# firstBusiness/mathmap

Measured on AMD Instinct MI355X. Metric: Mpixels/sec (mandelbrot @8192x8192), higher is better.
Workload: dtype f32

## Files before the change

### include/mmhip.h

```cpp
#ifndef MMHIP_H
#define MMHIP_H

#include <stddef.h>
#include <stdint.h>

#ifdef __cplusplus
extern "C" {
#endif

typedef struct mmhip_filter mmhip_filter;
typedef struct mmhip_invocation mmhip_invocation;

enum { MMHIP_UV_INT = 0, MMHIP_UV_FLOAT = 1, MMHIP_UV_BOOL = 2, MMHIP_UV_COLOR = 3,
       MMHIP_UV_CURVE = 4, MMHIP_UV_GRADIENT = 5, MMHIP_UV_IMAGE = 6 };

enum { MMHIP_EDGE_COLOR = 0, MMHIP_EDGE_WRAP = 1, MMHIP_EDGE_REFLECT = 2, MMHIP_EDGE_ROTATE = 3 };

enum { MMHIP_GAUSS_EXACT = 0, MMHIP_GAUSS_TOLERANCE = 1 };

typedef struct mmhip_options {
    int intersample;
    int supersampling;
    int edge_behaviour_x, edge_behaviour_y;
    int tile_w;
    int specialize_uservals;
    int pixel_inc;
    int gauss_mode;
    int reserved[5];
} mmhip_options;

typedef struct mmhip_userval_info {
    int kind;
    int index;
    char name[64];
    int int_min, int_max, int_default;
    float float_min, float_max, float_default;
    int bool_default;
    unsigned image_flags;
} mmhip_userval_info;

const char *mmhip_last_error(void);
const char *mmhip_version(void);

void mmhip_default_options(mmhip_options *o);
mmhip_filter *mmhip_compile(const char *source, const mmhip_options *opts);
mmhip_filter *mmhip_compile_specialized(const char *source, const mmhip_options *opts, int n, const int *indices,
                                        const double *values);
mmhip_filter *mmhip_filter_specialized(const mmhip_filter *f, int n, const int *indices, const double *values);
mmhip_filter *mmhip_compile_ir_json(const char *ir_json, const mmhip_options *opts);
void mmhip_filter_free(mmhip_filter *f);
const char *mmhip_filter_name(const mmhip_filter *f);
int mmhip_filter_num_uservals(const mmhip_filter *f);
int mmhip_filter_userval_info(const mmhip_filter *f, int index, mmhip_userval_info *out);
const char *mmhip_filter_ir_json(mmhip_filter *f);
const char *mmhip_filter_ir_json_raw(mmhip_filter *f);
const char *mmhip_filter_kernel_source(mmhip_filter *f);
int mmhip_filter_gauss_mode(const mmhip_filter *f);
int mmhip_filter_num_native_calls(const mmhip_filter *f);
int mmhip_filter_builtin_ids(const mmhip_filter *f, char *buf, int cap);
enum { MMHIP_GEOMETRY_FIELDS = 13 };
int mmhip_filter_launch_geometry(const mmhip_filter *f, int region_w, int num_rows, int64_t *out);
int mmhip_filter_num_closures(const mmhip_filter *f);
int mmhip_filter_closure_launch_geometry(const mmhip_filter *f, int closure, int width, int height, int64_t *out);
int mmhip_filter_clip_launch_geometry(const mmhip_filter *f, int region_w, int num_rows, int frames, int64_t *out);
enum { MMHIP_CLIP_PLAN_FIELDS = 4 };
int mmhip_filter_clip_batch_plan(const mmhip_filter *f, int region_w, int num_rows, int frames, int64_t *out);
enum { MMHIP_CLIP_NATIVE_PLAN_FIELDS = 4 };
int mmhip_filter_clip_native_plan(const mmhip_filter *f, int region_w, int num_rows, int render_w, int render_h, int frames,
                                  int64_t *out);
const char *mmhip_filter_clip_kernel_source(mmhip_filter *f);
long mmhip_filter_jit_clip(mmhip_filter *f, int load_module);
long mmhip_filter_jit(mmhip_filter *f, int load_module);
double mmhip_filter_jit_seconds(const mmhip_filter *f);

mmhip_invocation *mmhip_invoke(mmhip_filter *f, int img_width, int img_height);
void mmhip_invocation_free(mmhip_invocation *inv);
int mmhip_set_int(mmhip_invocation *inv, int index, int value);
int mmhip_set_float(mmhip_invocation *inv, int index, float value);
int mmhip_set_bool(mmhip_invocation *inv, int index, int value);
int mmhip_set_color(mmhip_invocation *inv, int index, float r, float g, float b, float a);
int mmhip_set_native_row_margin(mmhip_invocation *inv, int margin);
int mmhip_set_curve(mmhip_invocation *inv, int index, const float *values1024);
int mmhip_set_gradient(mmhip_invocation *inv, int index, const uint32_t *rgba1024);
int mmhip_set_by_name(mmhip_invocation *inv, const char *name, const char *value);
int mmhip_set_image_host(mmhip_invocation *inv, int index, const uint8_t *pixels, int width, int height, int channels);
int mmhip_set_image_device(mmhip_invocation *inv, int index, const void *device_rgba32, int width, int height);
int mmhip_set_image_sequence_host(mmhip_invocation *inv, int index, const uint8_t *pixels, int width, int height, int channels,
                                  int num_frames);
int mmhip_set_image_sequence_device(mmhip_invocation *inv, int index, const void *device_rgba32, int width, int height,
                                    int num_frames);
enum { MMHIP_NATIVE_FRAME_ZERO = 0, MMHIP_NATIVE_FRAME_CURRENT = 1 };
int mmhip_set_native_input_frame(mmhip_invocation *inv, int mode);
int mmhip_set_edge_colors(mmhip_invocation *inv, uint32_t color_x, uint32_t color_y);
int mmhip_set_render_size(mmhip_invocation *inv, int render_width, int render_height);
int mmhip_set_sampling_offset(mmhip_invocation *inv, float offset_x, float offset_y);

int mmhip_render(mmhip_invocation *inv, int frame, float t, int region_x, int region_y, int region_w, int region_h,
                 int first_row, int last_row, void *out_device, int row_stride, int bpp, int floatmap, void *stream);
int mmhip_render_clip(mmhip_invocation *inv, int num_frames, const int *frames, const float *ts, int region_x, int region_y,
                      int region_w, int region_h, int first_row, int last_row, void *out_device, int row_stride,
                      int64_t frame_stride, int bpp, int floatmap, void *stream);
long mmhip_clip_batched_launches(mmhip_invocation *inv);
long mmhip_clip_prologue_frames(mmhip_invocation *inv);
long mmhip_clip_native_batches(mmhip_invocation *inv);
long mmhip_clip_native_blurs(mmhip_invocation *inv);
long mmhip_clip_native_direct_frames(mmhip_invocation *inv);
int mmhip_render_supersampled(mmhip_invocation *inv, int frame, float t, int region_x, int region_y, int region_w,
                              int region_h, void *out_device, int row_stride, int bpp, void *stream);
int mmhip_render_clip_supersampled(mmhip_invocation *inv, int num_frames, const int *frames, const float *ts,
                                   int region_x, int region_y, int region_w, int region_h, void *out_device, int row_stride,
                                   int64_t frame_stride, int bpp, void *stream);
long mmhip_clip_supersampled_batches(mmhip_invocation *inv);
enum { MMHIP_CLIP_SS_PLAN_FIELDS = 7 };
int mmhip_filter_clip_supersample_plan(const mmhip_filter *f, int region_w, int region_h, int bpp, int frames, int64_t *out);
int mmhip_render_host(mmhip_invocation *inv, int frame, float t, uint8_t *out_rgba);
int mmhip_sync(mmhip_invocation *inv);
int mmhip_enable_timing(mmhip_invocation *inv, int on);
double mmhip_last_kernel_ms(mmhip_invocation *inv);
int mmhip_drain_kernel_ms(mmhip_invocation *inv, double *out_ms, int cap);
int mmhip_drain_native_kernel_ms(mmhip_invocation *inv, char *names, double *out_ms, int cap);
long mmhip_direct_native_launches(mmhip_invocation *inv);
long mmhip_tolerance_blur_launches(mmhip_invocation *inv);

void *mmhip_device_alloc(size_t bytes);
void mmhip_device_free(void *p);
int mmhip_copy_to_host(void *dst_host, const void *src_device, size_t bytes);
int mmhip_copy_to_device(void *dst_device, const void *src_host, size_t bytes);
int mmhip_device_count(void);
int mmhip_set_device(int ordinal);

#ifdef __cplusplus
}
#endif
#endif
```

### mathmap_amd/_lib.py

```python
import ctypes as C
import os

_HERE = os.path.dirname(os.path.abspath(__file__))
LIB_PATH = os.path.join(_HERE, "libmathmap_hip.so")


class Options(C.Structure):
    _fields_ = [("intersample", C.c_int), ("supersampling", C.c_int),
                ("edge_behaviour_x", C.c_int), ("edge_behaviour_y", C.c_int),
                ("tile_w", C.c_int), ("specialize_uservals", C.c_int), ("pixel_inc", C.c_int),
                ("gauss_mode", C.c_int), ("reserved", C.c_int * 5)]


class UservalInfo(C.Structure):
    _fields_ = [("kind", C.c_int), ("index", C.c_int), ("name", C.c_char * 64),
                ("int_min", C.c_int), ("int_max", C.c_int), ("int_default", C.c_int),
                ("float_min", C.c_float), ("float_max", C.c_float), ("float_default", C.c_float),
                ("bool_default", C.c_int), ("image_flags", C.c_uint)]


SYMBOLS = {
    "mmhip_last_error": (C.c_char_p, []),
    "mmhip_version": (C.c_char_p, []),
    "mmhip_default_options": (None, [C.POINTER(Options)]),
    "mmhip_compile": (C.c_void_p, [C.c_char_p, C.POINTER(Options)]),
    "mmhip_compile_specialized": (C.c_void_p, [C.c_char_p, C.POINTER(Options), C.c_int, C.POINTER(C.c_int),
                                               C.POINTER(C.c_double)]),
    "mmhip_compile_ir_json": (C.c_void_p, [C.c_char_p, C.POINTER(Options)]),
    "mmhip_filter_specialized": (C.c_void_p, [C.c_void_p, C.c_int, C.POINTER(C.c_int), C.POINTER(C.c_double)]),
    "mmhip_filter_free": (None, [C.c_void_p]),
    "mmhip_filter_name": (C.c_char_p, [C.c_void_p]),
    "mmhip_filter_num_uservals": (C.c_int, [C.c_void_p]),
    "mmhip_filter_userval_info": (C.c_int, [C.c_void_p, C.c_int, C.POINTER(UservalInfo)]),
    "mmhip_filter_ir_json": (C.c_char_p, [C.c_void_p]),
    "mmhip_filter_ir_json_raw": (C.c_char_p, [C.c_void_p]),
    "mmhip_filter_kernel_source": (C.c_char_p, [C.c_void_p]),
    "mmhip_filter_gauss_mode": (C.c_int, [C.c_void_p]),
    "mmhip_filter_num_native_calls": (C.c_int, [C.c_void_p]),
    "mmhip_filter_builtin_ids": (C.c_int, [C.c_void_p, C.c_char_p, C.c_int]),
    "mmhip_filter_launch_geometry": (C.c_int, [C.c_void_p, C.c_int, C.c_int, C.POINTER(C.c_int64)]),
    "mmhip_filter_clip_launch_geometry": (C.c_int, [C.c_void_p, C.c_int, C.c_int, C.c_int, C.POINTER(C.c_int64)]),
    "mmhip_filter_clip_batch_plan": (C.c_int, [C.c_void_p, C.c_int, C.c_int, C.c_int, C.POINTER(C.c_int64)]),
    "mmhip_filter_clip_native_plan": (C.c_int, [C.c_void_p, C.c_int, C.c_int, C.c_int, C.c_int, C.c_int, C.POINTER(C.c_int64)]),
    "mmhip_filter_clip_kernel_source": (C.c_char_p, [C.c_void_p]),
    "mmhip_filter_jit_clip": (C.c_long, [C.c_void_p, C.c_int]),
    "mmhip_filter_num_closures": (C.c_int, [C.c_void_p]),
    "mmhip_filter_closure_launch_geometry": (C.c_int, [C.c_void_p, C.c_int, C.c_int, C.c_int, C.POINTER(C.c_int64)]),
    "mmhip_filter_jit": (C.c_long, [C.c_void_p, C.c_int]),
    "mmhip_filter_jit_seconds": (C.c_double, [C.c_void_p]),
    "mmhip_invoke": (C.c_void_p, [C.c_void_p, C.c_int, C.c_int]),
    "mmhip_invocation_free": (None, [C.c_void_p]),
    "mmhip_set_int": (C.c_int, [C.c_void_p, C.c_int, C.c_int]),
    "mmhip_set_float": (C.c_int, [C.c_void_p, C.c_int, C.c_float]),
    "mmhip_set_bool": (C.c_int, [C.c_void_p, C.c_int, C.c_int]),
    "mmhip_set_color": (C.c_int, [C.c_void_p, C.c_int, C.c_float, C.c_float, C.c_float, C.c_float]),
    "mmhip_set_native_row_margin": (C.c_int, [C.c_void_p, C.c_int]),
    "mmhip_set_native_input_frame": (C.c_int, [C.c_void_p, C.c_int]),
    "mmhip_drain_kernel_ms": (C.c_int, [C.c_void_p, C.c_void_p, C.c_int]),
    "mmhip_direct_native_launches": (C.c_long, [C.c_void_p]),
    "mmhip_tolerance_blur_launches": (C.c_long, [C.c_void_p]),
    "mmhip_drain_native_kernel_ms": (C.c_int, [C.c_void_p, C.c_char_p, C.c_void_p, C.c_int]),
    "mmhip_set_curve": (C.c_int, [C.c_void_p, C.c_int, C.c_void_p]),
    "mmhip_set_gradient": (C.c_int, [C.c_void_p, C.c_int, C.c_void_p]),
    "mmhip_set_by_name": (C.c_int, [C.c_void_p, C.c_char_p, C.c_char_p]),
    "mmhip_set_image_host": (C.c_int, [C.c_void_p, C.c_int, C.c_void_p, C.c_int, C.c_int, C.c_int]),
    "mmhip_set_image_device": (C.c_int, [C.c_void_p, C.c_int, C.c_void_p, C.c_int, C.c_int]),
    "mmhip_set_image_sequence_host": (C.c_int, [C.c_void_p, C.c_int, C.c_void_p, C.c_int, C.c_int, C.c_int, C.c_int]),
    "mmhip_set_image_sequence_device": (C.c_int, [C.c_void_p, C.c_int, C.c_void_p, C.c_int, C.c_int, C.c_int]),
    "mmhip_set_edge_colors": (C.c_int, [C.c_void_p, C.c_uint32, C.c_uint32]),
    "mmhip_set_render_size": (C.c_int, [C.c_void_p, C.c_int, C.c_int]),
    "mmhip_set_sampling_offset": (C.c_int, [C.c_void_p, C.c_float, C.c_float]),
    "mmhip_render": (C.c_int, [C.c_void_p, C.c_int, C.c_float, C.c_int, C.c_int, C.c_int, C.c_int,
                               C.c_int, C.c_int, C.c_void_p, C.c_int, C.c_int, C.c_int, C.c_void_p]),
    "mmhip_render_clip": (C.c_int, [C.c_void_p, C.c_int, C.POINTER(C.c_int), C.POINTER(C.c_float), C.c_int, C.c_int, C.c_int,
                                    C.c_int, C.c_int, C.c_int, C.c_void_p, C.c_int, C.c_int64, C.c_int, C.c_int, C.c_void_p]),
    "mmhip_clip_batched_launches": (C.c_long, [C.c_void_p]),
    "mmhip_clip_prologue_frames": (C.c_long, [C.c_void_p]),
    "mmhip_clip_native_batches": (C.c_long, [C.c_void_p]),
    "mmhip_clip_native_blurs": (C.c_long, [C.c_void_p]),
    "mmhip_clip_native_direct_frames": (C.c_long, [C.c_void_p]),
    "mmhip_render_supersampled": (C.c_int, [C.c_void_p, C.c_int, C.c_float, C.c_int, C.c_int, C.c_int, C.c_int,
                                            C.c_void_p, C.c_int, C.c_int, C.c_void_p]),
    "mmhip_render_clip_supersampled": (C.c_int, [C.c_void_p, C.c_int, C.POINTER(C.c_int), C.POINTER(C.c_float), C.c_int, C.c_int,
                                                 C.c_int, C.c_int, C.c_void_p, C.c_int, C.c_int64, C.c_int, C.c_void_p]),
    "mmhip_clip_supersampled_batches": (C.c_long, [C.c_void_p]),
    "mmhip_filter_clip_supersample_plan": (C.c_int, [C.c_void_p, C.c_int, C.c_int, C.c_int, C.c_int, C.POINTER(C.c_int64)]),
    "mmhip_render_host": (C.c_int, [C.c_void_p, C.c_int, C.c_float, C.c_void_p]),
    "mmhip_sync": (C.c_int, [C.c_void_p]),
    "mmhip_enable_timing": (C.c_int, [C.c_void_p, C.c_int]),
    "mmhip_last_kernel_ms": (C.c_double, [C.c_void_p]),
    "mmhip_device_alloc": (C.c_void_p, [C.c_size_t]),
    "mmhip_device_free": (None, [C.c_void_p]),
    "mmhip_copy_to_host": (C.c_int, [C.c_void_p, C.c_void_p, C.c_size_t]),
    "mmhip_copy_to_device": (C.c_int, [C.c_void_p, C.c_void_p, C.c_size_t]),
    "mmhip_device_count": (C.c_int, []),
    "mmhip_set_device": (C.c_int, [C.c_int]),
}

BACKEND_SYMBOLS = {
    "gen_and_load_hip_code": (C.c_void_p, [C.c_void_p, C.POINTER(C.c_void_p), C.c_char_p, C.c_char_p, C.c_void_p]),
    "unload_hip_code": (None, [C.c_void_p]),
    "mathmap_hip_set_get_pixel": (None, [C.c_void_p]),
    "mathmap_hip_invalidate_drawable": (None, [C.c_void_p]),
    "mathmap_hip_release_invocation": (None, [C.c_void_p]),
}

SELFTEST_SYMBOLS = {
    "mmhip_selftest_abi_roundtrip": (C.c_int, [C.c_char_p, C.c_int, C.c_void_p, C.c_int, C.c_int, C.c_int, C.c_int,
                                               C.c_int, C.c_float, C.c_int, C.c_void_p]),
    "mmhip_selftest_error": (C.c_char_p, []),
    "mmhip_selftest_set_pixel_inc": (None, [C.c_int]),
    "mmhip_selftest_eval_unary": (C.c_int, [C.c_int, C.c_uint, C.c_ulonglong, C.c_void_p]),
    "mmhip_selftest_eval_binary": (C.c_int, [C.c_int, C.c_ulonglong, C.c_ulonglong, C.c_void_p]),
    "mmhip_selftest_gauss_tolerance_map": (C.c_int, [C.c_void_p, C.c_int, C.c_int, C.c_float, C.c_float, C.c_void_p]),
    "mmhip_selftest_combine_ms": (C.c_long, [C.c_int, C.c_int, C.c_int, C.c_int, C.c_int, C.POINTER(C.c_double)]),
}
SELFTEST_PATH = os.path.join(_HERE, "libmathmap_hip_selftest.so")
_selftest = None


def selftest_lib():
    global _selftest
    if _selftest is None:
        lib()
        l = C.CDLL(SELFTEST_PATH, mode=C.RTLD_GLOBAL)
        for name, (res, args) in SELFTEST_SYMBOLS.items():
            fn = getattr(l, name)
            fn.restype = res
            fn.argtypes = args
        _selftest = l
    return _selftest

_lib = None


def lib():
    global _lib
    if _lib is None:
        if not os.path.exists(LIB_PATH):
            raise ImportError(
                "%s is missing: build it with `python -c 'import __graft_entry__ as g; g.build()'` "
                "or `make -C mathmap_amd/csrc` (there is no CPU fallback)" % LIB_PATH)
        l = C.CDLL(LIB_PATH)
# ... 7 lines not shown
```

### mathmap_amd/api.py

```python
import ctypes as C
import json

import numpy as np

from ._lib import Options, UservalInfo, lib

UV_INT, UV_FLOAT, UV_BOOL, UV_COLOR, UV_CURVE, UV_GRADIENT, UV_IMAGE = range(7)
GAUSS_MODES = {"exact": 0, "tolerance": 1}
NATIVE_INPUT_FRAMES = {"zero": 0, "current": 1}
EDGE_COLOR, EDGE_WRAP, EDGE_REFLECT, EDGE_ROTATE = range(4)
GEOMETRY_FIELDS = ("tiles_x", "tiles_y", "wg1", "nwg", "ppt", "tile_w", "tile_h", "unroll", "pair_mode", "single_pixel",
                   "xcd_order", "tiles_magic", "xcd_full")
CLIP_PLAN_FIELDS = ("grid_x", "frames_per_batch", "batches", "shared_slot")
CLIP_NATIVE_PLAN_FIELDS = ("eligible", "frames_per_batch", "batches", "bytes_per_frame")
CLIP_SS_PLAN_FIELDS = ("batched", "frames_per_batch", "batches", "bytes_per_frame", "long_pitch", "rows_per_item", "pixels_per_item")


class MathMapError(RuntimeError):
    pass


def _err():
    return lib().mmhip_last_error().decode("utf-8", "replace")

# ... 26 lines not shown
        if not self._h:
            raise MathMapError(_err())
        if constants:
            base, self._h = self._h, None
            try:
                self._h = self._specialized_handle(base, constants)
            finally:
                lib().mmhip_filter_free(base)

    @staticmethod
    def _specialized_handle(handle, constants):
        names = {}
        for i in range(lib().mmhip_filter_num_uservals(handle)):
            info = UservalInfo()
            lib().mmhip_filter_userval_info(handle, i, C.byref(info))
            names[info.name.decode()] = i
        for k in constants:
            if k not in names:
                raise MathMapError("filter has no user value `%s'" % k)
        idx = (C.c_int * len(constants))(*[names[k] for k in constants])
        val = (C.c_double * len(constants))(*[float(v) for v in constants.values()])
        h = lib().mmhip_filter_specialized(handle, len(constants), idx, val)
        if not h:
            raise MathMapError(_err())
        return h

    def __del__(self):
        h, self._h = getattr(self, "_h", None), None
        if h:
            lib().mmhip_filter_free(h)

    @property
    def name(self):
        return lib().mmhip_filter_name(self._h).decode()

    @property
    def uservals(self):
        out = []
        for i in range(lib().mmhip_filter_num_uservals(self._h)):
            info = UservalInfo()
            lib().mmhip_filter_userval_info(self._h, i, C.byref(info))
            out.append(dict(kind=info.kind, index=info.index, name=info.name.decode(),
                            int_min=info.int_min, int_max=info.int_max, int_default=info.int_default,
                            float_min=info.float_min, float_max=info.float_max, float_default=info.float_default,
                            bool_default=info.bool_default, image_flags=info.image_flags))
        return out

    @property
    def ir(self):
        return json.loads(lib().mmhip_filter_ir_json(self._h).decode())

    @property
    def ir_json(self):
        return lib().mmhip_filter_ir_json(self._h).decode()

    @property
    def ir_json_raw(self):
        return lib().mmhip_filter_ir_json_raw(self._h).decode()

    def specialized(self, values=None):
        consts = {}
        for u in self.uservals:
            if u["kind"] == UV_INT:
                consts[u["name"]] = u["int_default"]
            elif u["kind"] == UV_FLOAT:
                consts[u["name"]] = u["float_default"]
            elif u["kind"] == UV_BOOL:
                consts[u["name"]] = u["bool_default"]
        for k, v in (values or {}).items():
            if k in consts:
                consts[k] = v
        return Filter(self._source, _handle=self._specialized_handle(self._h, consts), **self._kwargs)

    @property
    def kernel_source(self):
        return lib().mmhip_filter_kernel_source(self._h).decode()

    @property
    def gauss_mode(self):
        mode = lib().mmhip_filter_gauss_mode(self._h)
        return {v: k for k, v in GAUSS_MODES.items()}[mode]

    @property
    def num_native_calls(self):
        return lib().mmhip_filter_num_native_calls(self._h)

    @property
    def builtin_ids(self):
        n = lib().mmhip_filter_builtin_ids(self._h, None, 0)
        buf = C.create_string_buffer(n)
        lib().mmhip_filter_builtin_ids(self._h, buf, n)
        return frozenset(buf.value.decode().split())

    def launch_geometry(self, region_w, num_rows, closure=None):
        out = (C.c_int64 * len(GEOMETRY_FIELDS))()
        if closure is None:
            rc = lib().mmhip_filter_launch_geometry(self._h, region_w, num_rows, out)
        else:
            rc = lib().mmhip_filter_closure_launch_geometry(self._h, closure, region_w, num_rows, out)
        if rc != 0:
            raise MathMapError(_err())
        return dict(zip(GEOMETRY_FIELDS, out))

    def clip_launch_geometry(self, region_w, num_rows, frames):
        out = (C.c_int64 * len(GEOMETRY_FIELDS))()
        if lib().mmhip_filter_clip_launch_geometry(self._h, region_w, num_rows, frames, out) != 0:
            raise MathMapError(_err())
        return dict(zip(GEOMETRY_FIELDS, out))

    def clip_batch_plan(self, region_w, num_rows, frames):
        out = (C.c_int64 * len(CLIP_PLAN_FIELDS))()
        if lib().mmhip_filter_clip_batch_plan(self._h, region_w, num_rows, frames, out) != 0:
            raise MathMapError(_err())
        return dict(zip(CLIP_PLAN_FIELDS, out))

    def clip_native_plan(self, region_w, num_rows, frames, render_w=None, render_h=None):
        out = (C.c_int64 * len(CLIP_NATIVE_PLAN_FIELDS))()
        rw, rh = region_w if render_w is None else render_w, num_rows if render_h is None else render_h
        if lib().mmhip_filter_clip_native_plan(self._h, region_w, num_rows, rw, rh, frames, out) != 0:
            raise MathMapError(_err())
        return dict(zip(CLIP_NATIVE_PLAN_FIELDS, out))

    def clip_supersample_plan(self, region_w, region_h, frames, bpp=4):
        out = (C.c_int64 * len(CLIP_SS_PLAN_FIELDS))()
        if lib().mmhip_filter_clip_supersample_plan(self._h, region_w, region_h, bpp, frames, out) != 0:
            raise MathMapError(_err())
        return dict(zip(CLIP_SS_PLAN_FIELDS, out))

    @property
    def clip_kernel_source(self):
        return lib().mmhip_filter_clip_kernel_source(self._h).decode()

    def jit_clip(self, load=False):
        n = lib().mmhip_filter_jit_clip(self._h, 1 if load else 0)
        if n < 0:
            raise MathMapError(_err())
        return n

    @property
    def num_closures(self):
        return lib().mmhip_filter_num_closures(self._h)

    def jit(self, load=False):
        n = lib().mmhip_filter_jit(self._h, 1 if load else 0)
        if n < 0:
            raise MathMapError(_err())
        return n

    @property
    def jit_seconds(self):
        return lib().mmhip_filter_jit_seconds(self._h)

    def invoke(self, width, height):
        return Invocation(self, width, height)


def as_image_sequence(array):
    a = np.ascontiguousarray(array, dtype=np.uint8)
    if a.ndim == 3:
        a = a[None]
    if a.ndim != 4 or a.shape[0] < 1:
        raise MathMapError("an image is [H,W,3|4], an image sequence [N,H,W,3|4] with N >= 1; got shape %s" % (tuple(np.shape(array)),))
    return a


class Invocation:
# ... 26 lines not shown
        u = self._index(name)
        k, i = u["kind"], u["index"]
        if k == UV_INT:
            self._check(lib().mmhip_set_int(self._h, i, int(value)))
        elif k == UV_FLOAT:
            self._check(lib().mmhip_set_float(self._h, i, float(value)))
        elif k == UV_BOOL:
            self._check(lib().mmhip_set_bool(self._h, i, int(bool(value))))
        elif k == UV_COLOR:
            r, g, b, a = value
            self._check(lib().mmhip_set_color(self._h, i, r, g, b, a))
        elif k == UV_IMAGE:
            self.set_image(name, value)
        else:
            raise MathMapError("cannot set user value `%s'" % name)

    def set_curve(self, name, values):
        u = self._index(name)
        a = np.ascontiguousarray(values, dtype=np.float32)
        if a.shape != (1024,):
            raise MathMapError("a curve has 1024 samples")
        self._check(lib().mmhip_set_curve(self._h, u["index"], a.ctypes.data_as(C.c_void_p)))

    def set_gradient(self, name, rgba):
        u = self._index(name)
        a = np.ascontiguousarray(rgba, dtype=np.uint32)
        if a.shape != (1024,):
            raise MathMapError("a gradient has 1024 samples")
        self._check(lib().mmhip_set_gradient(self._h, u["index"], a.ctypes.data_as(C.c_void_p)))

    def set_image(self, name, array):
        u = self._index(name)
        a = as_image_sequence(array)
        n, h, w, c = a.shape
        self._check(lib().mmhip_set_image_sequence_host(self._h, u["index"], a.ctypes.data_as(C.c_void_p), w, h, c, n))

    def set_image_device(self, name, device_ptr, width, height, keepalive=None, num_frames=1):
        u = self._index(name)
        self._check(lib().mmhip_set_image_sequence_device(self._h, u["index"], C.c_void_p(device_ptr), width, height, num_frames))
        if keepalive is not None:
            self._keep.append(keepalive)

    def set_native_row_margin(self, margin):
        self._check(lib().mmhip_set_native_row_margin(self._h, margin))

    def set_native_input_frame(self, mode):
        if mode not in NATIVE_INPUT_FRAMES:
            raise MathMapError("native input frame must be one of %s, not %r" % (", ".join(sorted(NATIVE_INPUT_FRAMES)), mode))
        self._check(lib().mmhip_set_native_input_frame(self._h, NATIVE_INPUT_FRAMES[mode]))

    def set_render_size(self, render_width, render_height):
        self._check(lib().mmhip_set_render_size(self._h, render_width, render_height))
        self.render_width, self.render_height = render_width, render_height

    def set_edge_colors(self, cx, cy):
        self._check(lib().mmhip_set_edge_colors(self._h, cx, cy))

    def enable_timing(self, on=True):
        self._check(lib().mmhip_enable_timing(self._h, 1 if on else 0))

    def last_kernel_ms(self):
        return lib().mmhip_last_kernel_ms(self._h)

    def drain_kernel_ms(self, cap=4096):
        buf = (C.c_double * cap)()
        n = lib().mmhip_drain_kernel_ms(self._h, buf, cap)
        if n < 0:
            raise MathMapError(_err())
        return [buf[i] for i in range(n)]

    def drain_native_kernel_ms(self, cap=4096):
        names = C.create_string_buffer(cap * 64)
        buf = (C.c_double * cap)()
        n = lib().mmhip_drain_native_kernel_ms(self._h, names, buf, cap)
        if n < 0:
            raise MathMapError(_err())
        return [(names.raw[i * 64:(i + 1) * 64].split(b"\0", 1)[0].decode(), buf[i]) for i in range(n)]

    def direct_native_launches(self):
        return lib().mmhip_direct_native_launches(self._h)

    def tolerance_blur_launches(self):
        return lib().mmhip_tolerance_blur_launches(self._h)

    def render(self, t=0.0, frame=0):
        out = np.empty((self.render_height, self.render_width, 4), dtype=np.uint8)
        self._check(lib().mmhip_render_host(self._h, frame, t, out.ctypes.data_as(C.c_void_p)))
        return out

    def render_rows(self, out_ptr, first_row, last_row, t=0.0, frame=0, row_stride=None, bpp=4, floatmap=False,
                    stream=0, region=None):
        rx, ry, rw, rh = region if region is not None else (0, 0, self.render_width, self.render_height)
        if row_stride is None:
            row_stride = rw * bpp
        self._check(lib().mmhip_render(self._h, frame, t, rx, ry, rw, rh, first_row, last_row, C.c_void_p(out_ptr),
                                       row_stride, bpp, 1 if floatmap else 0, C.c_void_p(stream)))

    def render_clip(self, num_frames=None, frames=None, ts=None, out_ptr=None, rows=None, region=None, row_stride=None,
                    frame_stride=None, bpp=4, floatmap=False, stream=0, supersample=False):
        from .striping import animation_frame_t
        if supersample and (floatmap or rows is not None):
            raise ValueError("render_clip: supersample=True renders whole regions of bytes: neither floatmap nor rows")
        if frames is None and ts is None:
            if num_frames is None:
                raise MathMapError("render_clip: give num_frames, or frames and ts")
            frames = list(range(num_frames))
            ts = [animation_frame_t(i, num_frames) for i in frames]
        elif frames is None or ts is None:
            raise MathMapError("render_clip: frames and ts go together")
        frames = np.ascontiguousarray(frames, dtype=np.int32).reshape(-1)
        ts = np.ascontiguousarray(ts, dtype=np.float32).reshape(-1)
        if num_frames is None:
            num_frames = len(frames)
        if len(frames) != num_frames or len(ts) != num_frames:
            raise MathMapError("render_clip: frames and ts must have num_frames = %d entries" % num_frames)
        rx, ry, rw, rh = region if region is not None else (0, 0, self.render_width, self.render_height)
        first_row, last_row = rows if rows is not None else (ry, ry + rh)
        fp, tp = frames.ctypes.data_as(C.POINTER(C.c_int)), ts.ctypes.data_as(C.POINTER(C.c_float))
        if supersample:
            return self._render_clip_supersampled(num_frames, fp, tp, out_ptr, (rx, ry, rw, rh), row_stride, frame_stride, bpp, stream)
        if out_ptr is not None:
            if row_stride is None:
                row_stride = rw * bpp
            if frame_stride is None:
                n_rows = max(min(last_row, ry + rh) - max(first_row, 0), 0)
                frame_stride = n_rows * (16 * self.render_width if floatmap else row_stride)
            self._check(lib().mmhip_render_clip(self._h, num_frames, fp, tp, rx, ry, rw, rh, first_row, last_row,
                                                C.c_void_p(out_ptr), row_stride, frame_stride, bpp, 1 if floatmap else 0,
                                                C.c_void_p(stream)))
            return None
        if rows is not None or region is not None or floatmap or bpp != 4 or row_stride is not None or frame_stride is not None:
            raise MathMapError("render_clip without out_ptr returns whole RGBA frames: pass out_ptr for bands, regions and other formats")
        out = np.empty((num_frames, self.render_height, self.render_width, 4), dtype=np.uint8)
        if num_frames < 1:
            raise MathMapError("render_clip: num_frames must be at least 1")
        dev = lib().mmhip_device_alloc(out.nbytes)
        if not dev:
            raise MathMapError(_err())
        try:
            self._check(lib().mmhip_render_clip(self._h, num_frames, fp, tp, rx, ry, rw, rh, first_row, last_row,
                                                C.c_void_p(dev), rw * 4, rw * 4 * rh, 4, 0, None))
            self.sync()
            self._check(lib().mmhip_copy_to_host(out.ctypes.data_as(C.c_void_p), C.c_void_p(dev), out.nbytes))
        finally:
            lib().mmhip_device_free(C.c_void_p(dev))
        return out

    def _render_clip_supersampled(self, num_frames, fp, tp, out_ptr, region, row_stride, frame_stride, bpp, stream):
        rx, ry, rw, rh = region
        if row_stride is None:
            row_stride = rw * bpp
        if frame_stride is None:
            frame_stride = rh * row_stride
        if out_ptr is not None:
            self._check(lib().mmhip_render_clip_supersampled(self._h, num_frames, fp, tp, rx, ry, rw, rh, C.c_void_p(out_ptr),
                                                             row_stride, frame_stride, bpp, C.c_void_p(stream)))
            return None
        if row_stride != rw * bpp or frame_stride != rh * rw * bpp:
            raise MathMapError("render_clip without out_ptr returns packed frames: pass out_ptr for padded rows and frames")
        if num_frames < 1:
            raise MathMapError("render_clip: num_frames must be at least 1")
        out = np.empty((num_frames, rh, rw, bpp), dtype=np.uint8)
        dev = lib().mmhip_device_alloc(out.nbytes)
        if not dev:
            raise MathMapError(_err())
        try:
# ... 42 lines not shown
```

### mathmap_amd/csrc/hipgen.cpp

```cpp
#include <cmath>
#include <cstdio>
#include <cstdlib>
#include <cstring>
#include <map>
#include <set>
#include <sstream>
#include <stdexcept>

#include "front.h"
#include "hipgen_internal.h"

namespace mm {
namespace hipgen {

std::optional<int> env_int(const char *name) {
    const char *e = getenv(name);
    return e ? std::optional<int>(atoi(e)) : std::nullopt;
}

std::string vname(const Value *v) {
    char buf[64];
    snprintf(buf, sizeof buf, "v%d_%d", v->var->id, v->index);
    return buf;
}
// ... 295 lines not shown
                    collect_values(s->phis, sl, defs, uses);
                    use(s->cond);
                    collect_values(s->body, sl, defs, uses);
                    break;
                default: break;
            }
        }
    }

    template <class F> static void each_stmt(const Block &b, F f) {
        for (const Stmt *s : b) {
            if (!f(s)) continue;
            if (s->kind == Stmt::If) { each_stmt(s->then_, f); each_stmt(s->else_, f); }
            if (s->kind == Stmt::While) each_stmt(s->body, f);
        }
    }
    static bool is_op(const Stmt *s, const char *cname, size_t n = 0) {
        return s->kind == Stmt::Assign && s->rhs.kind == Rhs::Op && (n ? !strncmp(s->rhs.op->cname, cname, n) : !strcmp(s->rhs.op->cname, cname));
    }
    static bool uses_noise(const Block &b) {
        bool noise = false;
        each_stmt(b, [&](const Stmt *s) { noise = noise || is_op(s, "libnoise_", 9); return true; });
        return noise;
    }

    std::string site_desc(const Stmt *s) const {
        auto it = site_view.find(s);
        return it != site_view.end() ? it->second : vname(s->rhs.args[2].value) + "_desc";
    }
    const Stmt *find_fetched_result() const {
        if (!opt.intersample || knobs.no_fetched_result) return nullptr;
        const Stmt *fetch = nullptr;
        for (int i = 0; i < 4; ++i) {
            const Value *v = code.result[i];
            const Stmt *d = v ? v->def : nullptr;
            if (!d || d->kind != Stmt::Assign || d->parent || !d->in_pixel || d->rhs.kind != Rhs::Op || strcmp(d->rhs.op->cname, "TUPLE_NTH") ||
                d->rhs.args[0].kind != Primary::Val || d->rhs.args[1].kind != Primary::IntConst || d->rhs.args[1].i != i)
                return nullptr;
            const Stmt *f = d->rhs.args[0].value->def;
            if (!f || f->parent || !(hot_sites.count(f) || hot_frame_sites.count(f)) || (fetch && f != fetch)) return nullptr;
            fetch = f;
        }
        return fetch;
    }

    void find_hot_fetches(const Block &b, std::vector<std::string> &views, std::vector<std::string> &conds) {
        std::vector<const Stmt *> sites;
        each_stmt(b, [&](const Stmt *s) {
            if (s->in_pixel && is_op(s, "ORIG_VAL") && s->rhs.args.size() == 4 && s->rhs.args[2].kind == Primary::Val && preloaded_desc.count(s->rhs.args[2].value))
                sites.push_back(s);
            return s->in_pixel;
        });
        auto frame_const = [&](const Primary &f) { return f.is_const() || (f.kind == Primary::Val && transfer_off.count(f.value)); };
        std::map<const Value *, std::set<std::string>> frames_of;
        for (const Stmt *s : sites)
            if (frame_const(s->rhs.args[3])) frames_of[s->rhs.args[2].value].insert(prim(s->rhs.args[3], PIXEL));
        const bool frame_hot = knobs.frame_hot.value_or(1) != 0;
        for (const Stmt *s : sites) {
            const Primary &f = s->rhs.args[3];
            const std::string desc = vname(s->rhs.args[2].value) + "_desc";
            if (frame_const(f)) {
                hot_sites.insert(s);
                if (frames_of[s->rhs.args[2].value].size() > 1) {
                    const std::string view = "mm_fv" + std::to_string(site_view.size());
                    views.push_back("const mm_image_desc " + view + " = mm_frame_view(" + desc + ");");
                    site_view[s] = view;
                }
                conds.push_back("mm_fetch_is_hot(" + site_desc(s) + ", (int)(" + prim(f, PIXEL) + "))");
            } else if (frame_hot) {
                hot_frame_sites.insert(s);
                conds.push_back("mm_fetch_is_hot_any(" + desc + ")");
            }
        }
    }

    static bool hoisted_uses_time(const Block &b) {
        bool uses = false;
        each_stmt(b, [&](const Stmt *s) {
            uses = uses || (s->hoisted && s->kind == Stmt::Assign && s->rhs.kind == Rhs::Internal && (s->rhs.internal == "t" || s->rhs.internal == "frame"));
            return true;
        });
        return uses;
    }
    static void pixel_stats(const Block &b, int &stmts, int &fetches) {
        each_stmt(b, [&](const Stmt *s) { stmts += s->in_pixel; fetches += s->in_pixel && is_op(s, "ORIG_VAL"); return s->in_pixel; });
    }

    int auto_unroll() const {
        if (knobs.unroll && *knobs.unroll >= 1 && *knobs.unroll <= 8) return *knobs.unroll;
        if (pixel_fetches == 0) return 1;
        return pixel_stmts <= 64 ? 4 : pixel_stmts <= 400 ? 2 : 1;
    }
    int auto_tile_w() const { return pixel_fetches >= 1 && pixel_stmts <= 12 ? 64 : 16; }

    void find_natives(Block &b, int loop_depth = 0) {
        for (Stmt *s : b) {
            if (s->kind == Stmt::Assign) {
                bool native = (s->rhs.kind == Rhs::Closure && s->rhs.filter->kind == Filter::Native) ||
                              (s->rhs.kind == Rhs::Op && !strcmp(s->rhs.op->cname, "RENDER"));
                if (native) {
                    NativeCall nc;
                    nc.func = s->rhs.kind == Rhs::Closure ? s->rhs.filter->native_func : "RENDER";
                    for (const Primary &p : s->rhs.args) nc.arg_types.push_back(p.type());
                    nc.in_loop = loop_depth > 0;
                    native_index[s] = (int)ks.natives.size();
                    ks.natives.push_back(nc);
                }
            } else if (s->kind == Stmt::If) {
                find_natives(s->then_, loop_depth);
                find_natives(s->else_, loop_depth);
            } else if (s->kind == Stmt::While)
                find_natives(s->body, loop_depth + 1);
        }
    }

    void phis(Block &list, int branch, Slice sl, const std::string &ind) {
        auto src = [&](const Stmt *p) -> const Rhs & { return branch == 0 ? p->rhs : p->rhs2; };
        auto src_value = [&](const Stmt *p) { return src(p).kind == Rhs::Prim && src(p).prim.kind == Primary::Val ? src(p).prim.value : nullptr; };
        std::vector<Stmt *> mine;
        std::set<Value *> targets;
        for (Stmt *p : list)
            if (p->kind == Stmt::Phi && (sl == PROLOGUE ? p->hoisted : p->in_pixel) && src_value(p) != p->lhs) { mine.push_back(p); targets.insert(p->lhs); }
        bool hazard = false;
        for (Stmt *p : mine) hazard = hazard || targets.count(src_value(p)) > 0;
        if (!hazard) {
            for (Stmt *p : mine) out << ind << vname(p->lhs) << " = " << rhs(src(p), sl, p, p->lhs->var) << ";\n";
            return;
        }
        out << ind << "{\n";
        for (size_t i = 0; i < mine.size(); ++i)
            out << ind << "  " << ctype(mine[i]->lhs->var) << " pc" << i << " = "
                << rhs(src(mine[i]), sl, mine[i], mine[i]->lhs->var) << ";\n";
        for (size_t i = 0; i < mine.size(); ++i) out << ind << "  " << vname(mine[i]->lhs) << " = pc" << i << ";\n";
        out << ind << "}\n";
    }

    static bool is_sin_or_cos(const Stmt *s, bool *is_sin) {
        if (s->kind != Stmt::Assign || s->rhs.kind != Rhs::Op || s->rhs.args.size() != 1) return false;
        const char *cn = s->rhs.op->cname;
        if (strcmp(cn, "sin") && strcmp(cn, "cos")) return false;
        if (!s->lhs || s->lhs->var->type != Ty::Float || s->rhs.args[0].type() != Ty::Float || s->rhs.args[0].kind != Primary::Val)
            return false;
        *is_sin = !strcmp(cn, "sin");
        return true;
    }
    void join_sincos(Block &b) {
        for (size_t i = 0; i < b.size(); ++i) {
            bool sin_i, sin_j;
            Stmt *si = b[i];
            if (!si->in_pixel || sincos_role.count(si) || !is_sin_or_cos(si, &sin_i)) continue;
            for (size_t j = i + 1; j < b.size(); ++j) {
                Stmt *sj = b[j];
                if (!sj->in_pixel || sincos_role.count(sj) || !is_sin_or_cos(sj, &sin_j)) continue;
                if (sin_j == sin_i || sj->rhs.args[0].value != si->rhs.args[0].value) continue;
                sincos_role[si] = SinCosRole{sincos_ids, true};
                sincos_role[sj] = SinCosRole{sincos_ids, false};
                ++sincos_ids;
                break;
            }
        }
    }

    void stmts(Block &b, Slice sl, const std::string &ind) {
        if (opt.fast_math_exact && sl == PIXEL && sincos_scanned.insert(&b).second) join_sincos(b);
        for (Stmt *s : b) {
            bool mine = sl == PROLOGUE ? s->hoisted : sl == ROWS ? s->in_row : s->in_pixel;
// ... 285 lines not shown
}
struct mm_narg_t { int kind; int i; float f; mm_image img; };
MM_DEV mm_narg_t mm_narg(int v) { mm_narg_t a; a.kind = 0; a.i = v; a.f = (float)v; a.img = mm_null_image(); return a; }
MM_DEV mm_narg_t mm_narg(float v) { mm_narg_t a; a.kind = 1; a.i = (int)v; a.f = v; a.img = mm_null_image(); return a; }
MM_DEV mm_narg_t mm_narg(double v) { return mm_narg((float)v); }
MM_DEV mm_narg_t mm_narg(mm_image v) { mm_narg_t a; a.kind = 2; a.i = v.idx; a.f = 0.0f; a.img = v; return a; }
// Records a native-filter call for the host (which runs the filter's kernels between
// the prologue and the pixel kernel) and returns the handle of its result float map.
// ctr[0] counts the calls of this frame in the order they are made (the host runs them in that order).
MM_DEV mm_image mm_native_call(const mm_args &A, char *rec, int *ctr, int k, int nargs, mm_narg_t a0, mm_narg_t a1, mm_narg_t a2, mm_narg_t a3) {
    int *hdr = (int *)rec;
    hdr[0] = 1; hdr[1] = k; hdr[2] = nargs; hdr[3] = ctr[0]++;
    mm_narg_t *args = (mm_narg_t *)(rec + 16);
    args[0] = a0; args[1] = a1; args[2] = a2; args[3] = a3;
    mm_image im; im.idx = A.native_slot_base + k; im.pw = A.render_width; im.ph = A.render_height;
    im.xf = im.yf = 1.0f; im.resized = 0;
    return im;
}
// The same for a call site inside a loop: every call takes the next of the MM_NATIVE_DYN_CALLS dynamic entries behind
// the `sites' call sites (record, result slot); one call too many raises ctr[2] and the host refuses the frame.
MM_DEV mm_image mm_native_call_in_loop(const mm_args &A, char *dyn, int *ctr, int site, int sites, int nargs, mm_narg_t a0, mm_narg_t a1,
                                       mm_narg_t a2, mm_narg_t a3) {
    int n = ctr[1]++;
    if (n >= MM_NATIVE_DYN_CALLS) { ctr[2] = 1; n = MM_NATIVE_DYN_CALLS - 1; }
    mm_image im = mm_native_call(A, dyn + n * MM_NATIVE_REC_BYTES, ctr, site, nargs, a0, a1, a2, a3);
    im.idx = A.native_slot_base + sites + n;
    return im;
}
// (float) frame column / row of the pixel being evaluated (render_image's per-pixel loop, builtins.c:324-333)
#define __colF ((float)(col + A.region_x))
#define __rowF ((float)(rl + A.first_row))
#define MM_INTERNALS \
    const float t = A.t; const float R = A.R; const int frame = A.frame; \
    const int __canvasPixelW = A.img_width, __canvasPixelH = A.img_height; \
    const int __renderPixelW = A.render_width, __renderPixelH = A.render_height; \
    (void)t; (void)R; (void)frame; (void)__canvasPixelW; (void)__canvasPixelH; (void)__renderPixelW; (void)__renderPixelH;
)";
        if (ks.native_sites < (int)ks.natives.size())
            out << R"(// The pixel slice's side of a loop that runs in both slices: its n-th call from an in-loop site is the prologue's n-th.
MM_DEV mm_image mm_native_result_in_loop(const mm_args &A, int &n, int sites) {
    mm_image im; im.idx = A.native_slot_base + sites + (n < MM_NATIVE_DYN_CALLS ? n : MM_NATIVE_DYN_CALLS - 1); ++n;
    im.pw = A.render_width; im.ph = A.render_height; im.xf = im.yf = 1.0f; im.resized = 0;
    return im;
}
)";
    }

    void emit_functions() {
        FilterCode &root = fn_root ? *fn_root : code;
        if (root.functions.empty()) return;
        out << "#ifndef MM_MAX_CALL_DEPTH\n#define MM_MAX_CALL_DEPTH " << knobs.max_call_depth.value_or(16)
            << "\n#endif\n"
               "struct mm_uvarg { int i; float f; color_t c; mm_image img; };\n";
        auto head = [](size_t k) {
            return "template <int MM_D> __device__ __noinline__ mm_tup<4> mm_filter_" + std::to_string(k) +
                   "(const mm_args &A, const mm_uvarg *UV, float x, float y, float t, int col, int rl, unsigned &mm_rand_ctr)";
        };
        for (size_t k = 0; k < root.functions.size(); ++k) out << head(k) << ";\n";
        for (size_t k = 0; k < root.functions.size(); ++k) {
            FilterCode &fn = *root.functions[k];
            Generator g(fn, opt, knobs);
            g.fn_root = &root;
            g.in_function = true;
            std::vector<Value *> defs;
            std::set<Value *> uses;
            g.collect_values(fn.body, PIXEL, defs, uses);
            out << "// filter_" << (fn.filter ? fn.filter->name : "") << "\n" << head(k) << " {\n"
                   "  mm_tup<4> rt;\n  rt.v[0] = rt.v[1] = rt.v[2] = rt.v[3] = 0.0f;\n"
                   "  if constexpr (MM_D >= MM_MAX_CALL_DEPTH) { return rt; } else {\n"
                   "  const float R = A.R; const int frame = 0;      // new_template.c.in:379: filter_$name has `int frame = 0`\n"
                   "  const int __canvasPixelW = A.img_width, __canvasPixelH = A.img_height;\n"
                   "  const int __renderPixelW = A.render_width, __renderPixelH = A.render_height;\n"
                   "  (void)R; (void)frame; (void)__canvasPixelW; (void)__canvasPixelH; (void)__renderPixelW; (void)__renderPixelH;\n";
            g.decls(defs, "  ");
            g.stmts(fn.body, PIXEL, "  ");
            out << g.out.str();
            for (int i = 0; i < 4; ++i) out << "  rt.v[" << i << "] = " << g.prim(Primary::V(fn.result[i]), PIXEL) << ";\n";
            out << "  return rt;\n  }\n}\n";
        }
    }

    void emit_prologue_kernel() {
        ks.prologue_uses_time = hoisted_uses_time(code.body);
        ks.prologue_name = "mm_prologue";
        ks.pixel_name = "mm_pixels";
        auto tables = [](const std::string &first) {
            return "  {\n    const int gid = blockIdx.x * 256 + threadIdx.x;\n"
                   "    if (" + first + "gid < A.region_width) A.xtab[gid] = CALC_VIRTUAL_X(gid + A.region_x, A.frame_render_width, A.sampling_offset_x);\n"
                   "    if (" + first + "gid < A.num_rows) A.ytab[gid] = CALC_VIRTUAL_Y(A.first_row + gid, A.frame_render_height, A.sampling_offset_y);\n"
                   "    if (gid != 0) return;\n  }\n";
        };
        emit(KERNEL + "mm_prologue(mm_args A, char *XY) {\n" + tables(""),
             (ks.natives.empty() ? clip_prelude() : clip_prelude_natives()) + KERNEL + "mm_prologue_clip(mm_args A, char *XY, const mm_clip C) {\n  MM_CLIP_ENTRY\n" + tables("fi == 0 && "));
        out << "  MM_INTERNALS\n";
        if (!(fn_root ? fn_root : &code)->functions.empty()) out << "  const int col = 0, rl = 0; unsigned mm_rand_ctr = 0; (void)col; (void)rl; (void)mm_rand_ctr;\n";
        decls(pro_defs, "  ", true);
        if (!ks.natives.empty()) {
            for (const NativeCall &nc : ks.natives) out << "  *(int *)(XY + " << nc.record_offset << ") = 0;\n";
            out << "  { int *mm_ctr = (int *)(XY + " << ks.native_ctr_offset << "); mm_ctr[0] = mm_ctr[1] = mm_ctr[2] = mm_ctr[3] = 0; }\n";
        }
        stmts(code.body, PROLOGUE, "  ");
        for (Value *v : transfer_order)
            out << "  *(" << ctype(v->var) << " *)(XY + " << transfer_off[v] << ") = " << vname(v) << ";\n";
        out << "}\n\n";
    }

    void emit_rows_kernel() {
        emit(KERNEL + "mm_rows(mm_args A, const char *__restrict__ XY) {\n",
             KERNEL + "mm_rows_clip(mm_args A, const char *__restrict__ XY, const mm_clip C) {\n  MM_CLIP_ENTRY\n");
        out << "  const int rl = blockIdx.x * 256 + threadIdx.x;\n"
               "  if (rl >= A.num_rows) return;\n"
               "  MM_INTERNALS\n"
               "  const float y = A.ytab[rl];    // CALC_VIRTUAL_Y(first_row + rl, ...), by the prologue\n"
               "  (void)y;\n";
        transfer_loads(&row_uses);
        decls(row_defs, "  ");
        stmts(code.body, ROWS, "  ");
        for (size_t k = 0; k < row_transfer.size(); ++k) {
            Value *v = row_transfer[k];
            out << "  A.rowtab[" << k << " * A.num_rows + rl] = "
                << (v->var->type == Ty::Int ? "__int_as_float(" + vname(v) + ")" : vname(v)) << ";\n";
        }
        out << "}\n\n";
    }

    void emit_pixel_kernel() {
        if (knobs.waves_per_eu) out << "__attribute__((amdgpu_waves_per_eu(" << *knobs.waves_per_eu << "))) ";
        emit(KERNEL + "mm_pixels(mm_args A, const char *__restrict__ XY) {\n",
             KERNEL + "mm_pixels_clip(mm_args A, const char *__restrict__ XY, const mm_clip C) {\n"
                      "  if ((int)blockIdx.x >= C.nwg) return;      // padding workgroup\n  MM_CLIP_ENTRY\n");
        out << R"(  MM_INTERNALS
  // XCD-aware tile order (MM_XCD_ORDER, above): workgroups are dealt round-robin to the 8 XCDs; give each
  // XCD one contiguous band of tiles so neighbouring gathers share its L2 -- or, for a kernel that reads nothing,
  // take the tiles in dispatch order so that cheap and expensive regions of the frame are spread over all XCDs.
  const int tiles_x = (A.region_width + MM_TILE_W - 1) / MM_TILE_W;
)";
        emit("  const int nwg = gridDim.x;\n", "  const int nwg = C.nwg;      // the frame's workgroups (gridDim.x is padded)\n");
        out << R"(  const int bid = blockIdx.x;
#if MM_XCD_ORDER == 1
  const int xcd = bid & 7, q = bid >> 3;
  const int per = nwg >> 3, rem = nwg & 7;
  const int swz = xcd * per + (xcd < rem ? xcd : rem) + q;
#elif MM_XCD_ORDER == 2
  // runs of C = 2^m consecutive tiles (m: one tile row or a little more) dealt to the XCDs in turn: neighbours in a row
  // share an L2 like in a band, and every XCD gets runs from all over the frame; the last partial round keeps dispatch order
  const int m = 32 - __builtin_clz((unsigned)(tiles_x > 1 ? tiles_x - 1 : 1));
  const int full = (nwg >> (m + 3)) << (m + 3);
  const int q = bid >> 3;
  const int swz = bid < full ? ((((q >> m) << 3) + (bid & 7)) << m) + (q & ((1 << m) - 1)) : bid;
#else
  const int swz = bid;
  (void)nwg;
#endif
  const int tile_y = A.tiles_magic ? (int)__umulhi((unsigned)swz, A.tiles_magic) : swz / tiles_x, tile_x = swz - tile_y * tiles_x;
  const int col = tile_x * MM_TILE_W + (threadIdx.x % MM_TILE_W);
  // a workgroup owns MM_TILE_W x (MM_TILE_H * A.ppt) pixels; each work-item walks A.ppt rows
  // MM_TILE_H apart, so wave start-up (kernarg / descriptor loads, tile arithmetic) and the
  // dispatcher's per-workgroup cost are paid once per A.ppt pixels
  const int row0 = tile_y * (MM_TILE_H * A.ppt) + (threadIdx.x / MM_TILE_W);   // row within this launch
  if (col >= A.region_width) return;
  const float x = A.xtab[col];   // CALC_VIRTUAL_X(col + region_x, ...), once per column
  (void)x;
)";
        transfer_loads(nullptr);
        ks.single_pixel = knobs.single_pixel ? *knobs.single_pixel != 0 : pixel_stmts > 400 || transfer_order.size() > 24;
        if (ks.single_pixel) emit_single_pixel();
// ... 147 lines not shown
```

### mathmap_amd/csrc/hipgen.h

```cpp
#pragma once
#include <string>
#include <vector>

#include "ir.h"

namespace mm {

struct KernelOptions {
    int intersample = 1;
    int supersampling = 0;
    int edge_x = 0, edge_y = 0;
    int pixel_inc = 1;
    int tile_w = 0;
    int unroll = 0;
    bool hoist = true;
    bool fast_math_exact = true;
};

struct NativeCall {
    std::string func;
    std::vector<Ty> arg_types;
    int record_offset = 0;
    bool in_loop = false;
    bool dynamic = false;
};

enum { MM_NATIVE_REC_BYTES = 320, MM_NATIVE_ARG_BYTES = 32, MM_NATIVE_MAX_ARGS = 9, MM_NATIVE_DYN_CALLS = 16 };

struct KernelSource {
    std::string source;
    std::string prologue_name, pixel_name;
    int xy_bytes = 0;
    bool has_prologue = false;
    std::vector<NativeCall> natives;
    int native_sites = 0;
    int native_ctr_offset = -1;
    int tile_w = 16, tile_h = 16;
    int unroll = 1;
    bool prologue_uses_time = true;
    bool single_pixel = false;
    bool pair_mode = false;
    bool pair_exit = false;
    int xcd_order = 2;
    int row_values = 0;
    std::string rows_name;
    int direct_native = -1;
    std::string key;
    struct Splice { size_t begin, end; std::string text; };
    std::vector<Splice> clip_splices;
};

KernelSource generate_hip(FilterCode &code, const KernelOptions &opt, FilterCode *functions_of = nullptr);
bool pair_peel_enabled();
void clip_kernel_source(const KernelSource &ks, std::string *source, std::string *key);
const char *clip_prelude();
const char *clip_prelude_natives();
const char *device_prelude();
const char *device_noise_prelude();
const char *device_fastmath_prelude();
const char *noise_table_text();

}
```

### mathmap_amd/csrc/native_filters.h

```cpp
#pragma once
#include <hip/hip_runtime.h>

#include <string>
#include <vector>

#include "mm_host_abi.h"

namespace mm {

struct NativeEnv {
    int supersampling = 0;
    int edge_x = 0, edge_y = 0;
    uint32_t edge_color_x = 0, edge_color_y = 0;
};

struct NativeWorkspace {
    NativeEnv env;
    bool gauss_tolerance = false;
    void *scratch = nullptr;
    size_t scratch_bytes = 0;
    bool keep_tolerance_map = false;
    void *reserve(size_t bytes);
    void release();
    struct Timed { const char *name; hipEvent_t a, b; };
    bool timing = false;
    std::vector<Timed> timed;
    std::vector<std::pair<hipEvent_t, hipEvent_t>> timed_free;
    template <class F> void timed_launch(const char *name, hipStream_t s, F &&launch) {
        if (!timing || timed.size() >= 4096) { launch(); return; }
        Timed t{name, nullptr, nullptr};
        if (!timed_free.empty()) { t.a = timed_free.back().first; t.b = timed_free.back().second; timed_free.pop_back(); }
        else if (hipEventCreate(&t.a) != hipSuccess || hipEventCreate(&t.b) != hipSuccess) { launch(); return; }
        (void)hipEventRecord(t.a, s);
        launch();
        (void)hipEventRecord(t.b, s);
        timed.push_back(t);
    }
    void *fft_fwd = nullptr, *fft_inv = nullptr;
    int fft_w = 0, fft_h = 0, fft_batch = 0;
    bool fft_valid = false;
};

struct NativeDirectOut {
    void *out = nullptr;
    int row_stride = 0;
    int first_row = 0, num_rows = 0, region_x = 0, region_w = 0;
    bool skip_map = false;
    bool written = false;
    bool tolerance = false;
};

int run_native_filter(const std::string &func, const HNativeRec &rec, const std::vector<HImageDesc> &images,
                      int render_w, int render_h, float *out_map, NativeWorkspace &ws, hipStream_t stream,
                      std::string *err, int *row_lo, int *row_hi,
                      NativeDirectOut *direct = nullptr);

bool gaussian_blur_batchable(const HNativeRec &rec, const HImageDesc *images, int num_images, int render_w, int render_h,
                             const NativeEnv &env, size_t *ckpt_bytes, size_t *map_bytes);
void gaussian_blur_batch_job_bytes(int render_w, int render_h, size_t *ckpt_bytes, size_t *map_bytes);
struct GaussClipJob {
    HNativeRec rec;
    const HImageDesc *images;
    int num_images;
    double *ckpt;
    float *mapT;
    float *out_map;
    unsigned char *pack_out;
};
struct GaussClipLaunch {
    int render_w = 0, render_h = 0;
    const NativeDirectOut *direct = nullptr;
    bool write_map = true;
};
size_t gaussian_blur_batch_table_bytes(size_t jobs);
struct GaussClipGroup { bool drawable; unsigned jobs; const void *vertical, *horizontal; unsigned pitch; };
int gaussian_blur_batch_tables(const std::vector<GaussClipJob> &jobs, const GaussClipLaunch &launch, const NativeEnv &env,
                               char *host_table, const char *device_table, std::vector<GaussClipGroup> *groups, std::string *err);
int gaussian_blur_batch_launch(const std::vector<GaussClipGroup> &groups, const GaussClipLaunch &launch, NativeWorkspace &ws,
                               hipStream_t s, std::string *err);

int fft_native_filter(const std::string &func, const HNativeRec &rec, const std::vector<HImageDesc> &images, int render_w,
                      int render_h, float *out_map, NativeWorkspace &ws, hipStream_t stream, std::string *err);
int native_input_map(const char *who, const HImage &img, const std::vector<HImageDesc> &images, const NativeEnv &env, int w,
                     int h, float *dst, const float **map, hipStream_t s, std::string *err);
void fft_release_plans(NativeWorkspace &ws);
void launch_render_drawable(const HImageDesc &in, const HImage &img, const NativeEnv &env, float *dst, int w, int h, hipStream_t s);

void launch_supersample_combine(const unsigned char *longs, const unsigned char *shorts, unsigned char *out, int w, int h,
                                int bpp, int out_stride, hipStream_t s);
constexpr int SS_CLIP_ROWS = 8, SS_CLIP_PIXELS = 4;
size_t supersample_clip_long_pitch(int w, int bpp);
int64_t supersample_clip_items(int w, int h);
int launch_supersample_combine_clip(const unsigned char *longs, const unsigned char *shorts, unsigned char *out, int w, int h,
                                    int bpp, int row_stride, int64_t frame_stride, int frames, NativeWorkspace &ws, hipStream_t s,
                                    std::string *err);

}
```

### mathmap_amd/csrc/native_filters.hip

```cpp
#include "native_filters.h"
#include "mm_ss_combine.h"

#include <algorithm>
#include <cmath>
#include <cstring>
#include <type_traits>
#include <vector>

namespace mm {

void *NativeWorkspace::reserve(size_t bytes) {
    if (bytes > scratch_bytes) {
        if (scratch) (void)hipFree(scratch);
        scratch = nullptr;
        if (hipMalloc(&scratch, bytes) != hipSuccess) { scratch_bytes = 0; return nullptr; }
        scratch_bytes = bytes;
    }
    return scratch;
}

void NativeWorkspace::release() {
    fft_release_plans(*this);
    for (Timed &t : timed) timed_free.push_back({t.a, t.b});
    timed.clear();
// ... 671 lines not shown
}

__device__ __forceinline__ long fir_index(const FirArgs &g, int line, int k, int ch) {
    return g.vertical ? ((long)k * g.w + line) * 4 + ch : ((long)line * g.w + k) * 4 + ch;
}

__global__ void __launch_bounds__(256) k_fir_same(const float *__restrict__ in, int *__restrict__ flags, FirArgs g) {
    const long L = (long)blockIdx.x * 256 + threadIdx.x;
    const int lines = g.vertical ? g.w : g.h, n = g.vertical ? g.h : g.w;
    if (L >= (long)lines * 4) return;
    const int line = (int)(L >> 2), ch = (int)(L & 3);
    float last = in[fir_index(g, line, n - 1, ch)];
    int same = 0;
    for (int k = n - 1; k >= 0; --k) {
        const float c = in[fir_index(g, line, k, ch)];
        if (c == last) same++;
        else last = c;
    }
    flags[L] = same > (3 * n) / 4;
}

__global__ void __launch_bounds__(256) k_fir_apply(const float *__restrict__ in, float *__restrict__ out,
                                                   const int *__restrict__ flags, const float *__restrict__ curve,
                                                   const float *__restrict__ csum, FirArgs g) {
    const long e = (long)blockIdx.x * 256 + threadIdx.x;
    if (e >= (long)g.w * g.h * 4) return;
    const int ch = (int)(e & 3);
    const long px = e >> 2;
    const int col = (int)(px % g.w), row = (int)(px / g.w);
    const int line = g.vertical ? col : row, k = g.vertical ? row : col;
    const int n = g.vertical ? g.h : g.w;
    const int length = g.length;
    const float *c = curve + length, *cs = csum + length;
    auto pix = [&](int i) {
        int kk = k + i;
        kk = kk < 0 ? 0 : (kk >= n ? n - 1 : kk);
        return in[fir_index(g, line, kk, ch)];
    };
    float val = 0.0f;
    if (!flags[line * 4 + ch]) {
        val += pix(0) * c[0];
        for (int i = 1; i <= length; ++i) val += (pix(i) + pix(-i)) * c[i];
        val = val / g.total;
    } else {
        int pos = -length;
        auto runlen = [&](int p) {
            const float v = pix(p);
            int r = 1;
            while (k + p + r < n + length && pix(p + r) == v) ++r;
            return r;
        };
        float s1 = cs[-length];
        int nb = runlen(pos);
        int i = -length + nb;
        while (i <= length) {
            const int s2 = (int)cs[i];
            val += pix(pos) * (s2 - s1);
            s1 = (float)s2;
            pos += nb;
            nb = runlen(pos);
            i += nb;
        }
        val += pix(pos) * (cs[length] - s1);
        val = val / g.ctotal;
    }
    out[e] = val;
}

int gauss_rle(float *map, float *tmp, int w, int h, float hs, float vs, NativeWorkspace &ws, char *aux, hipStream_t s,
              std::string *err) {
    float *src = map, *dst = tmp;
    for (int pass = 0; pass < 2; ++pass) {
        const int vertical = pass == 0;
        const float sd = vertical ? vs : hs;
        if (!(sd > 0.0f)) continue;
        std::vector<float> curve, sum;
        int length;
        float total;
        make_rle_curve(sd, curve, sum, length, total);
        const int lines = vertical ? w : h;
        int *flags = (int *)aux;
        float *d_curve = (float *)(aux + (size_t)std::max(w, h) * 4 * sizeof(int));
        float *d_sum = d_curve + curve.size();
        if (hipMemcpyAsync(d_curve, curve.data(), curve.size() * 4, hipMemcpyHostToDevice, s) != hipSuccess ||
            hipMemcpyAsync(d_sum, sum.data(), sum.size() * 4, hipMemcpyHostToDevice, s) != hipSuccess ||
            hipStreamSynchronize(s) != hipSuccess) {
            *err = "gaussian_blur: tap upload failed";
            return -1;
        }
        FirArgs g{w, h, vertical, length, total, (int)total};
        k_fir_same<<<(unsigned)(((long)lines * 4 + 255) / 256), 256, 0, s>>>(src, flags, g);
        k_fir_apply<<<(unsigned)(((long)w * h * 4 + 255) / 256), 256, 0, s>>>(src, dst, flags, d_curve, d_sum, g);
        std::swap(src, dst);
    }
    if (src != map && hipMemcpyAsync(map, src, (size_t)w * h * 16, hipMemcpyDeviceToDevice, s) != hipSuccess) {
        *err = "gaussian_blur: copy failed";
        return -1;
    }
    (void)ws;
    return 0;
}

struct GaussPlan {
    const HImageDesc *in = nullptr;
    int w = 0, h = 0;
    float hs = 0.f, vs = 0.f;
    bool fir = false;
    bool identity = false;
    size_t ckpt_bytes = 0;
    size_t scratch_bytes = 0;
    size_t map_bytes = 0;
};

size_t checkpoint_bytes(int w, int h) {
    const size_t ck_v = (size_t)((h + IIR_U - 1) / IIR_U) * 4 * ((size_t)w * 4) * sizeof(double);
    const size_t ck_h = (size_t)((w + IIR_U - 1) / IIR_U) * 4 * ((size_t)h * 4) * sizeof(double);
    return std::max(ck_v, ck_h);
}

bool scan_offsets_fit(int w, int hn) { return (long)std::max(w, hn) * 4 * 20 * 8 < (1L << 32); }

int plan_gaussian_blur(const HNativeRec &rec, const HImageDesc *images, int num_images, int rw, int rh, const NativeEnv &env,
                       GaussPlan *p, std::string *err) {
    const HImage &img = rec.args[0].img;
    const float hdev = rec.args[1].f, vdev = rec.args[2].f;
    if (img.idx < 0 || img.idx >= num_images) { *err = "gaussian_blur: input is not a bitmap image"; return -1; }
    const HImageDesc &in = images[img.idx];
    p->in = &in;
    int w = rw, h = rh;
    if (in.kind == IMG_FLOATMAP) {
        w = in.w;
        h = in.h;
        if (w != rw || h != rh) { *err = "gaussian_blur: float-map input of a different size is not supported"; return -1; }
    } else if (in.kind != IMG_DRAWABLE) {
        *err = "gaussian_blur: input image is not bound";
        return -1;
    }
    p->w = w;
    p->h = h;
    const float ax = (float)((float)(w - 1) / 2.0);
    float ay = (float)((float)(h - 1) / 2.0);
    ay *= -1.0f;
    p->hs = (float)fabs(hdev * ax);
    p->vs = (float)fabs(vdev * ay);
    p->ckpt_bytes = checkpoint_bytes(w, h);
    p->scratch_bytes = ((p->ckpt_bytes + (size_t)std::max(w, h) * 64 + (size_t)(w + h) * sizeof(int) + 65536) + 255) & ~(size_t)255;
    p->map_bytes = (size_t)w * h * 4 * sizeof(float);
    p->fir = p->hs < 0.5f || p->vs < 0.5f;
    bool identity = !p->fir && in.kind == IMG_DRAWABLE && in.w == w && in.h == h;
    if (identity) {
        const float ax = (float)((float)(w - 1) / 2.0), bx = ax;
        const float by = (float)((float)(h - 1) / 2.0);
        const float ay2 = (float)(by * -1.0);
        for (int i = 0; i < w && identity; ++i) {
            float x = ((float)i - bx) / ax;
            if (img.resized) x *= img.xf;
            x = (x + in.middle_x) * in.scale_x;
            if (!env.supersampling) x += 0.5;
            identity = (int)floor((double)x) == i;
        }
        for (int i = 0; i < h && identity; ++i) {
            float y = ((float)i - by) / ay2;
            if (img.resized) y *= img.yf;
            y = -((y - in.middle_y) * in.scale_y);
            if (!env.supersampling) y += 0.5;
            identity = (int)floor((double)y) == i;
// ... 387 lines not shown
```

### mathmap_amd/csrc/runtime.cpp

```cpp
#include <hip/hip_runtime.h>
#include <hip/hiprtc.h>
#include <sys/stat.h>
#include <unistd.h>

#include <algorithm>
#include <chrono>
#include <cmath>
#include <cstdio>
#include <cstdlib>
#include <cstring>
#include <fstream>
#include <map>
#include <memory>
#include <sstream>
#include <string>
#include <vector>

#include "../../include/mmhip.h"
#include "front.h"
#include "hipgen.h"
#include "mm_host_abi.h"
#include "native_filters.h"
#include "passes.h"
#include "runtime_internal.h"
// ... 104 lines not shown
mmhip_filter *mmhip_compile(const char *source, const mmhip_options *opts) { return compile_source(source, opts, nullptr); }

mmhip_filter *mmhip_compile_specialized(const char *source, const mmhip_options *opts, int n, const int *indices,
                                        const double *values) {
    Module probe;
    try {
        parse_module(probe, source);
    } catch (const std::exception &e) {
        g_err = e.what();
        return nullptr;
    }
    std::map<int, Primary> consts;
    for (int i = 0; i < n; ++i) {
        if (indices[i] < 0 || indices[i] >= (int)probe.main->uservals.size()) { g_err = "user value index out of range"; return nullptr; }
        const UservalInfo &u = probe.main->uservals[indices[i]];
        if (u.kind == UvKind::Float) consts[u.index] = Primary::F((float)values[i]);
        else if (u.kind == UvKind::Int || u.kind == UvKind::Bool) consts[u.index] = Primary::I((int)values[i]);
    }
    return compile_source(source, opts, &consts);
}

}

mmhip_filter *mmhip_filter_new_empty() { return new mmhip_filter(); }

bool mmhip_filter_finalize(mmhip_filter *f, const KernelOptions &ko, std::string *err) {
    try {
        f->code->filter = f->module.main;
        if (f->ir_json_raw.empty()) f->ir_json_raw = dump_ir(*f->code);
        optimize(*f->code);
        analyze_frame_constants(*f->code);
        for (auto &sub : f->code->closure_renders) {
            sub->filter = f->module.main;
            optimize(*sub);
            eliminate_dead_cycles(*sub);
            analyze_frame_constants(*sub);
        }
        for (auto &fn : f->code->functions) optimize(*fn);
        f->kopt = ko;
        f->ir_json = dump_ir(*f->code);
        f->ks = generate_hip(*f->code, ko);
        generate_closure_kernels(f, ko);
    } catch (const std::exception &e) {
        *err = e.what();
        return false;
    }
    return true;
}

extern "C" {

void mmhip_filter_free(mmhip_filter *f) {
    if (!f) return;
    for (auto &p : f->spec_cache) mmhip_filter_free(p.second);
    for (mmhip_closure_kernel &ck : f->closures) if (ck.mod) (void)hipModuleUnload(ck.mod);
    if (f->mod) (void)hipModuleUnload(f->mod);
    if (f->clip_mod) (void)hipModuleUnload(f->clip_mod);
    delete f;
}

const char *mmhip_filter_name(const mmhip_filter *f) { return f->module.main->name.c_str(); }
int mmhip_filter_num_uservals(const mmhip_filter *f) { return (int)f->module.main->uservals.size(); }

int mmhip_filter_userval_info(const mmhip_filter *f, int index, mmhip_userval_info *out) {
    const auto &uvs = f->module.main->uservals;
    if (index < 0 || index >= (int)uvs.size()) return fail("user value index out of range");
    const UservalInfo &u = uvs[index];
    memset(out, 0, sizeof *out);
    out->kind = (int)u.kind;
    out->index = u.index;
    snprintf(out->name, sizeof out->name, "%s", u.name.c_str());
    out->int_min = u.imin; out->int_max = u.imax; out->int_default = u.idef;
    out->float_min = u.fmin; out->float_max = u.fmax; out->float_default = u.fdef;
    out->bool_default = u.bdef;
    out->image_flags = u.image_flags;
    return 0;
}

const char *mmhip_filter_ir_json(mmhip_filter *f) { return f->ir_json.c_str(); }
const char *mmhip_filter_ir_json_raw(mmhip_filter *f) { return f->ir_json_raw.c_str(); }
const char *mmhip_filter_kernel_source(mmhip_filter *f) { return f->ks.source.c_str(); }
int mmhip_filter_gauss_mode(const mmhip_filter *f) { return f->opts.gauss_mode; }
int mmhip_filter_num_native_calls(const mmhip_filter *f) { return f->ks.native_sites; }

int mmhip_filter_builtin_ids(const mmhip_filter *f, char *buf, int cap) {
    std::string s;
    for (const std::string &id : f->module.resolved_ids) { s += id; s += '\n'; }
    if (buf && cap > 0) snprintf(buf, (size_t)cap, "%s", s.c_str());
    return (int)s.size() + 1;
}
double mmhip_filter_jit_seconds(const mmhip_filter *f) { return f->jit_seconds; }

static int jit_source(const KernelSource &ks, std::vector<char> &code_object) {
    if (!code_object.empty()) return 0;
    std::vector<std::string> extra;
    std::string extra_key;
    if (const char *e = getenv("MMHIP_HIPRTC_FLAGS")) {
        std::istringstream is(e);
        for (std::string w; is >> w;) { extra.push_back(w); extra_key += "_" + std::to_string(std::hash<std::string>()(w) & 0xffff); }
    }
    std::string path = cache_dir() + "/" + ks.key + "_o2" + extra_key + ".hsaco";
    std::ifstream in(path, std::ios::binary);
    const char *ov = getenv("MMHIP_SOURCE_OVERRIDE");
    const bool may_override = ov && !strncmp(ov, ks.key.c_str(), ks.key.size()) && ov[ks.key.size()] == ':';
    if (in && !getenv("MMHIP_NO_CACHE") && !may_override) code_object.assign(std::istreambuf_iterator<char>(in), std::istreambuf_iterator<char>());
    if (!code_object.empty()) return 0;
    std::string source = ks.source;
    bool overridden = false;
    if (const char *e = getenv("MMHIP_SOURCE_OVERRIDE")) {
        const std::string spec = e;
        const size_t c = spec.find(':');
        if (c != std::string::npos && spec.substr(0, c) == ks.key) {
            std::ifstream f(spec.substr(c + 1));
            if (!f) return fail("MMHIP_SOURCE_OVERRIDE: cannot read " + spec.substr(c + 1));
            source.assign(std::istreambuf_iterator<char>(f), std::istreambuf_iterator<char>());
            overridden = true;
        }
    }
    hiprtcProgram prog;
    if (hiprtcCreateProgram(&prog, source.c_str(), "mathmap_filter.hip", 0, nullptr, nullptr) != HIPRTC_SUCCESS)
        return fail("hiprtcCreateProgram failed");
    std::vector<const char *> opts = {"--offload-arch=gfx950", "-O3", "-ffp-contract=off", "-std=c++17", "-fno-slp-vectorize"};
    for (const std::string &w : extra) opts.push_back(w.c_str());
    hiprtcResult r = hiprtcCompileProgram(prog, (int)opts.size(), opts.data());
    if (r != HIPRTC_SUCCESS) {
        size_t n = 0;
        hiprtcGetProgramLogSize(prog, &n);
        std::string log(n, 0);
        if (n) hiprtcGetProgramLog(prog, &log[0]);
        hiprtcDestroyProgram(&prog);
        return fail("hiprtc compile failed:\n" + log);
    }
    size_t n = 0;
    hiprtcGetCodeSize(prog, &n);
    code_object.resize(n);
    hiprtcGetCode(prog, code_object.data());
    hiprtcDestroyProgram(&prog);
    if (overridden) return 0;
    std::string tmp = path + ".tmp" + std::to_string((int)getpid());
    std::ofstream o(tmp, std::ios::binary);
    if (o) {
        o.write(code_object.data(), (std::streamsize)code_object.size());
        o.close();
        rename(tmp.c_str(), path.c_str());
    }
    return 0;
}

static int load_kernels(const KernelSource &ks, const std::vector<char> &code_object, hipModule_t *mod, hipFunction_t *f_pix,
                        hipFunction_t *f_pro) {
    hipError_t e = hipModuleLoadData(mod, code_object.data());
    if (e != hipSuccess) return fail(std::string("hipModuleLoadData: ") + hipGetErrorString(e));
    e = hipModuleGetFunction(f_pix, *mod, ks.pixel_name.c_str());
    if (e != hipSuccess) return fail(std::string("hipModuleGetFunction(pixels): ") + hipGetErrorString(e));
    e = hipModuleGetFunction(f_pro, *mod, ks.prologue_name.c_str());
    if (e != hipSuccess) return fail(std::string("hipModuleGetFunction(prologue): ") + hipGetErrorString(e));
    return 0;
}

long mmhip_filter_jit(mmhip_filter *f, int load_module) {
    auto t0 = std::chrono::steady_clock::now();
    if (jit_source(f->ks, f->code_object) != 0) return -1;
    for (mmhip_closure_kernel &ck : f->closures)
        if (jit_source(ck.ks, ck.code_object) != 0) return -1;
    if (load_module && !f->loaded) {
        if (load_kernels(f->ks, f->code_object, &f->mod, &f->f_pix, &f->f_pro) != 0) return -1;
// ... 20 lines not shown
        f->clip_ks.pixel_name = "mm_pixels_clip";
    }
    return f->clip_ks;
}

const char *mmhip_filter_clip_kernel_source(mmhip_filter *f) { return clip_source(f).source.c_str(); }

long mmhip_filter_jit_clip(mmhip_filter *f, int load_module) {
    auto t0 = std::chrono::steady_clock::now();
    const mm::KernelSource &ks = clip_source(f);
    if (jit_source(ks, f->clip_code_object) != 0) return -1;
    if (load_module && !f->clip_loaded) {
        if (load_kernels(ks, f->clip_code_object, &f->clip_mod, &f->f_pix_clip, &f->f_pro_clip) != 0) return -1;
        if (f->ks.row_values > 0) {
            hipError_t e = hipModuleGetFunction(&f->f_rows_clip, f->clip_mod, ks.rows_name.c_str());
            if (e != hipSuccess) return fail(std::string("hipModuleGetFunction(rows): ") + hipGetErrorString(e));
        }
        f->clip_loaded = true;
    }
    f->jit_seconds += std::chrono::duration<double>(std::chrono::steady_clock::now() - t0).count();
    return (long)f->clip_code_object.size();
}

mmhip_invocation *mmhip_invoke(mmhip_filter *f, int img_width, int img_height) {
    if (img_width <= 0 || img_height <= 0) { fail("image size must be positive"); return nullptr; }
    if (mmhip_filter_jit(f, 1) < 0) return nullptr;
    std::unique_ptr<mmhip_invocation> inv(new mmhip_invocation());
    inv->f = f;
    inv->img_w = inv->render_w = img_width;
    inv->img_h = inv->render_h = img_height;
    const auto &uvs = f->module.main->uservals;
    inv->uv.resize(std::max<size_t>(uvs.size(), 1));
    inv->image_slot_of_uv.assign(uvs.size(), -1);
    HImageDesc null_desc{};
    null_desc.kind = IMG_NULL;
    for (const UservalInfo &u : uvs) {
        HUserval &v = inv->uv[u.index];
        v.i = 0;
        switch (u.kind) {
            case UvKind::Int: v.i = u.idef; break;
            case UvKind::Float: v.f = u.fdef; break;
            case UvKind::Bool: v.i = u.bdef ? 1 : 0; break;
            case UvKind::Color: v.c = 0x000000ffu; break;
            case UvKind::Curve: {
                v.i = (int)(inv->curves.size() / 1024);
                for (int i = 0; i < 1024; ++i) inv->curves.push_back((float)i / (float)(1024 - 1));
                break;
            }
            case UvKind::Gradient: {
                v.i = (int)(inv->gradients.size() / 1024);
                for (int i = 0; i < 1024; ++i) {
                    float g = (float)i / (float)(1024 - 1);
                    uint32_t q = (uint32_t)(int)(g * 255.0) & 0xff;
                    inv->gradients.push_back((q << 24) | (q << 16) | (q << 8) | 255u);
                }
                break;
            }
            case UvKind::Image: {
                int slot = (int)inv->images.size();
                inv->image_slot_of_uv[u.index] = slot;
                inv->images.push_back(null_desc);
                v.image = slot;
                break;
            }
        }
    }
    inv->native_slot_base = (int)inv->images.size();
    inv->natives.resize(f->ks.natives.size());
    inv->images.resize(inv->images.size() + inv->natives.size(), null_desc);
    inv->closure_state.resize(f->closures.size());
    for (size_t c = 0; c < f->closures.size(); ++c) {
        auto &st = inv->closure_state[c];
        st.native_slot_base = (int)inv->images.size();
        st.native_results.resize(f->closures[c].ks.natives.size());
        inv->images.resize(inv->images.size() + st.native_results.size(), null_desc);
    }
    if (inv->images.empty()) inv->images.push_back(null_desc);
    auto bail = [&](const char *what, hipError_t e) -> mmhip_invocation * {
        fail(std::string(what) + ": " + hipGetErrorString(e));
        return nullptr;
    };
    hipError_t e;
    if ((e = hipStreamCreate(&inv->stream.s)) != hipSuccess) return bail("hipStreamCreate", e);
    if ((e = inv->d_uv.grow(inv->uv.size() * sizeof(HUserval))) != hipSuccess) return bail("hipMalloc", e);
    if ((e = inv->d_images.grow(inv->images.size() * sizeof(HImageDesc))) != hipSuccess) return bail("hipMalloc", e);
    if ((e = inv->d_curves.grow(inv->curves.size() * 4)) != hipSuccess) return bail("hipMalloc", e);
    if ((e = inv->d_gradients.grow(inv->gradients.size() * 4)) != hipSuccess) return bail("hipMalloc", e);
    const int xy_bytes = std::max(f->ks.xy_bytes, 256);
    if ((e = inv->launch.xy.grow(xy_bytes, DeviceBuffer::no_wait, true)) != hipSuccess) return bail("hipMalloc", e);
    return inv.release();
}

mmhip_invocation::~mmhip_invocation() {
    if (stream) (void)hipStreamSynchronize(stream);
    ws.release();
    for (auto &p : ev_pool) {
        (void)hipEventDestroy(p.first);
        (void)hipEventDestroy(p.second);
    }
}

void mmhip_invocation_free(mmhip_invocation *inv) { delete inv; }

static const UservalInfo *uv_info(mmhip_invocation *inv, int index, UvKind kind) {
    const auto &uvs = inv->f->module.main->uservals;
    if (index < 0 || index >= (int)uvs.size()) { fail("user value index out of range"); return nullptr; }
    if (uvs[index].kind != kind) { fail("user value `" + uvs[index].name + "' has a different type"); return nullptr; }
    return &uvs[index];
}

int mmhip_set_int(mmhip_invocation *inv, int index, int value) {
    const UservalInfo *u = uv_info(inv, index, UvKind::Int);
    if (!u) return -1;
    inv->uv[index].i = value;
    inv->tables_dirty = true;
    return 0;
}

int mmhip_set_float(mmhip_invocation *inv, int index, float value) {
    const UservalInfo *u = uv_info(inv, index, UvKind::Float);
    if (!u) return -1;
    inv->uv[index].f = value;
    inv->tables_dirty = true;
    return 0;
}

int mmhip_set_bool(mmhip_invocation *inv, int index, int value) {
    const UservalInfo *u = uv_info(inv, index, UvKind::Bool);
    if (!u) return -1;
    inv->uv[index].i = value ? 1 : 0;
    inv->tables_dirty = true;
    return 0;
}

int mmhip_set_color(mmhip_invocation *inv, int index, float r, float g, float b, float a) {
    const UservalInfo *u = uv_info(inv, index, UvKind::Color);
    if (!u) return -1;
    auto q = [](float v) { v = v < 0 ? 0 : v > 1 ? 1 : v; return (uint32_t)(v * 255.0); };
    inv->uv[index].c = (q(r) << 24) | (q(g) << 16) | (q(b) << 8) | q(a);
    inv->tables_dirty = true;
    return 0;
}

int mmhip_set_by_name(mmhip_invocation *inv, const char *name, const char *value) {
    for (const UservalInfo &u : inv->f->module.main->uservals) {
        if (u.name != name) continue;
        switch (u.kind) {
            case UvKind::Int: return mmhip_set_int(inv, u.index, atoi(value));
            case UvKind::Float: return mmhip_set_float(inv, u.index, (float)atof(value));
            case UvKind::Bool: return mmhip_set_bool(inv, u.index, atoi(value));
            default: return fail(std::string("user value `") + name + "' cannot be set from a string");
        }
    }
    return fail(std::string("filter has no user value `") + name + "'");
}

static void fill_drawable_desc(HImageDesc &d, const void *data, int w, int h, int num_frames) {
    d.data = data;
    d.w = w;
    d.h = h;
    d.kind = IMG_DRAWABLE;
    d.num_frames = num_frames;
    d.scale_x = (float)((w - 1) / 2.0);
    d.scale_y = (float)((h - 1) / 2.0);
    d.middle_x = 1.0f;
    d.middle_y = 1.0f;
    d.ax = d.bx = d.ay = d.by = 0.f;
}

static HImageDesc floatmap_desc(const void *data, int w, int h) {
    HImageDesc d{};
    d.data = data;
    d.w = w;
    d.h = h;
    d.kind = IMG_FLOATMAP;
    d.num_frames = 1;
    d.ax = d.bx = (float)((float)(w - 1) / 2.0);
    d.ay = d.by = (float)((float)(h - 1) / 2.0);
    d.ay *= -1.0f;
    return d;
}

static void input_changed(mmhip_invocation *inv) {
    inv->tables_dirty = true;
    ++inv->input_generation;
}

static bool sequence_bytes(int width, int height, int num_frames, size_t &bytes) {
    if (width < 0 || height < 0 || num_frames < 1) return false;
    size_t texels = 0;
    if ((uint64_t)height * (uint64_t)num_frames > (uint64_t)INT32_MAX) return false;
    return !__builtin_mul_overflow((size_t)width, (size_t)height, &texels) && !__builtin_mul_overflow(texels, (size_t)num_frames, &texels) &&
           !__builtin_mul_overflow(texels, (size_t)4, &bytes) && bytes <= (size_t)PTRDIFF_MAX;
}

int mmhip_set_image_sequence_device(mmhip_invocation *inv, int index, const void *device_rgba32, int width, int height, int num_frames) {
    if (num_frames < 1) return fail("num_frames must be at least 1");
    size_t bytes = 0;
    if (!sequence_bytes(width, height, num_frames, bytes)) return fail("image sequence: the size overflows (fewer than 2^31 rows in all, and a byte count that fits)");
    const UservalInfo *u = uv_info(inv, index, UvKind::Image);
    if (!u) return -1;
    int slot = inv->image_slot_of_uv[index];
    fill_drawable_desc(inv->images[slot], device_rgba32, width, height, num_frames);
    input_changed(inv);
    return 0;
}

int mmhip_set_image_device(mmhip_invocation *inv, int index, const void *device_rgba32, int width, int height) {
    return mmhip_set_image_sequence_device(inv, index, device_rgba32, width, height, 1);
}

}

void mmhip_unbind_image(mmhip_invocation *inv, const void *data) {
    for (HImageDesc &img : inv->images)
        if (img.data == data) {
            img.kind = IMG_NULL;
            img.data = nullptr;
            input_changed(inv);
        }
}

extern "C" {

int mmhip_set_image_sequence_host(mmhip_invocation *inv, int index, const uint8_t *pixels, int width, int height, int channels,
                                  int num_frames) {
    if (channels != 3 && channels != 4) return fail("channels must be 3 or 4");
    if (num_frames < 1) return fail("num_frames must be at least 1");
    size_t bytes = 0;
    if (!sequence_bytes(width, height, num_frames, bytes)) return fail("image sequence: the size overflows (fewer than 2^31 rows in all, and a byte count that fits)");
    if (!uv_info(inv, index, UvKind::Image)) return -1;
    const size_t n = (size_t)width * height;
    std::vector<uint32_t> packed;
    try { packed.resize(n); } catch (const std::bad_alloc &) { return fail("image sequence: out of host memory"); }
    DeviceBuffer d;
    HIP_TRY(d.grow(bytes));
    for (int k = 0; k < num_frames; ++k) {
        const uint8_t *frame = pixels + (size_t)k * n * channels;
        for (size_t i = 0; i < n; ++i) {
            const uint8_t *p = frame + i * channels;
            uint32_t a = channels == 4 ? p[3] : 255u;
            packed[i] = ((uint32_t)p[0] << 24) | ((uint32_t)p[1] << 16) | ((uint32_t)p[2] << 8) | a;
        }
        HIP_TRY(hipMemcpy((char *)d.get() + (size_t)k * n * 4, packed.data(), n * 4, hipMemcpyHostToDevice));
    }
    const void *old = inv->images[inv->image_slot_of_uv[index]].data;
    for (auto it = inv->owned.begin(); it != inv->owned.end(); ++it)
        if (it->get() == old) {
            (void)hipDeviceSynchronize();
            inv->owned.erase(it);
            break;
        }
    const void *dev = d.get();
    inv->owned.push_back(std::move(d));
    return mmhip_set_image_sequence_device(inv, index, dev, width, height, num_frames);
}

int mmhip_set_image_host(mmhip_invocation *inv, int index, const uint8_t *pixels, int width, int height, int channels) {
    return mmhip_set_image_sequence_host(inv, index, pixels, width, height, channels, 1);
}

int mmhip_set_curve(mmhip_invocation *inv, int index, const float *values1024) {
    if (!uv_info(inv, index, UvKind::Curve)) return -1;
    float *dst = &inv->curves[(size_t)inv->uv[index].i * 1024];
    if (memcmp(dst, values1024, 1024 * sizeof(float)) == 0) return 0;
    memcpy(dst, values1024, 1024 * sizeof(float));
    inv->tables_dirty = true;
    return 0;
}

int mmhip_set_gradient(mmhip_invocation *inv, int index, const uint32_t *rgba1024) {
    if (!uv_info(inv, index, UvKind::Gradient)) return -1;
    uint32_t *dst = &inv->gradients[(size_t)inv->uv[index].i * 1024];
    if (memcmp(dst, rgba1024, 1024 * sizeof(uint32_t)) == 0) return 0;
    memcpy(dst, rgba1024, 1024 * sizeof(uint32_t));
    inv->tables_dirty = true;
    return 0;
}

int mmhip_set_native_row_margin(mmhip_invocation *inv, int margin) {
    inv->native_row_margin = margin;
    return 0;
}

int mmhip_set_native_input_frame(mmhip_invocation *inv, int mode) {
    if (mode != MMHIP_NATIVE_FRAME_ZERO && mode != MMHIP_NATIVE_FRAME_CURRENT)
        return fail("native input frame: mode " + std::to_string(mode) + " is neither MMHIP_NATIVE_FRAME_ZERO (0) nor MMHIP_NATIVE_FRAME_CURRENT (1)");
    if (inv->native_input_frame != mode) ++inv->input_generation;
    inv->native_input_frame = mode;
    return 0;
}

int mmhip_set_edge_colors(mmhip_invocation *inv, uint32_t cx, uint32_t cy) {
    inv->edge_color_x = cx;
    inv->edge_color_y = cy;
    return 0;
}

int mmhip_set_render_size(mmhip_invocation *inv, int rw, int rh) {
    inv->render_w = rw;
    inv->render_h = rh;
    return 0;
}

int mmhip_set_sampling_offset(mmhip_invocation *inv, float ox, float oy) {
    inv->sampling_offset_x = ox;
    inv->sampling_offset_y = oy;
    return 0;
}

int mmhip_enable_timing(mmhip_invocation *inv, int on) {
    inv->timing = on != 0;
    inv->ws.timing = on != 0;
    return 0;
}

int mmhip_drain_native_kernel_ms(mmhip_invocation *inv, char *names, double *out_ms, int cap) {
    auto &tm = inv->ws.timed;
    if (!tm.empty() && hipEventSynchronize(tm.back().b) != hipSuccess) return fail("event sync failed");
    int n = 0;
    for (auto &t : tm) {
        float ms = 0;
        if (n < cap && hipEventElapsedTime(&ms, t.a, t.b) == hipSuccess) {
            snprintf(names + (size_t)n * 64, 64, "%s", t.name);
            out_ms[n++] = ms;
        }
        inv->ws.timed_free.push_back({t.a, t.b});
    }
    tm.clear();
    return n;
}

static int next_event_pair(mmhip_invocation *inv) {
    if (inv->ev_used == inv->ev_pool.size()) {
        if (inv->ev_pool.size() >= 4096) inv->ev_used = 0;
        else {
            hipEvent_t a, b;
            HIP_TRY(hipEventCreate(&a));
            HIP_TRY(hipEventCreate(&b));
            inv->ev_pool.push_back({a, b});
        }
    }
    inv->ev0 = inv->ev_pool[inv->ev_used].first;
    inv->ev1 = inv->ev_pool[inv->ev_used].second;
    ++inv->ev_used;
    return 0;
}

long mmhip_direct_native_launches(mmhip_invocation *inv) { return inv->direct_native_launches; }
long mmhip_tolerance_blur_launches(mmhip_invocation *inv) { return inv->tolerance_blur_launches; }

int mmhip_drain_kernel_ms(mmhip_invocation *inv, double *out_ms, int cap) {
    int n = 0;
    if (inv->ev_used > 0 && hipEventSynchronize(inv->ev_pool[inv->ev_used - 1].second) != hipSuccess) return fail("event sync failed");
    for (size_t i = 0; i < inv->ev_used && n < cap; ++i) {
        float ms = 0;
        if (hipEventElapsedTime(&ms, inv->ev_pool[i].first, inv->ev_pool[i].second) != hipSuccess) return fail("event elapsed failed");
        out_ms[n++] = ms;
    }
    inv->ev_used = 0;
    inv->ev_valid = false;
    return n;
}

double mmhip_last_kernel_ms(mmhip_invocation *inv) {
    if (!inv->ev_valid) return -1.0;
    if (hipEventSynchronize(inv->ev1) != hipSuccess) return -1.0;
    float ms = 0;
    if (hipEventElapsedTime(&ms, inv->ev0, inv->ev1) != hipSuccess) return -1.0;
    return ms;
}

static int upload_image_table(mmhip_invocation *inv, hipStream_t s) {
    HIP_TRY(hipStreamSynchronize(s));
    HIP_TRY(hipMemcpy(inv->d_images.get(), inv->images.data(), inv->images.size() * sizeof(HImageDesc), hipMemcpyHostToDevice));
    return 0;
}

static int upload_tables(mmhip_invocation *inv, hipStream_t s) {
    if (!inv->tables_dirty) return 0;
    if (upload_image_table(inv, s) != 0) return -1;
    HIP_TRY(hipMemcpy(inv->d_uv.get(), inv->uv.data(), inv->uv.size() * sizeof(HUserval), hipMemcpyHostToDevice));
    if (inv->d_curves) HIP_TRY(hipMemcpy(inv->d_curves.get(), inv->curves.data(), inv->curves.size() * 4, hipMemcpyHostToDevice));
    if (inv->d_gradients) HIP_TRY(hipMemcpy(inv->d_gradients.get(), inv->gradients.data(), inv->gradients.size() * 4, hipMemcpyHostToDevice));
    inv->tables_dirty = false;
    ++inv->table_generation;
    return 0;
}

struct LaunchGeometry {
    int tiles_x = 0, tiles_y = 0;
    long wg1 = 0;
    long nwg = 0;
    int ppt = 1;
    uint32_t tiles_magic = 0;
};

static int rows_per_item(long wgs) { return wgs >= 262144 ? 16 : wgs >= 131072 ? 8 : wgs >= 32768 ? 4 : wgs >= 8192 ? 2 : 1; }

static LaunchGeometry launch_geometry(const KernelSource &ks, int region_w, int num_rows) {
    LaunchGeometry g;
    g.tiles_x = (region_w + ks.tile_w - 1) / ks.tile_w;
    g.wg1 = (long)g.tiles_x * ((num_rows + ks.tile_h - 1) / ks.tile_h);
    int ppt = rows_per_item(g.wg1);
    if (const char *e = getenv("MMHIP_PPT")) ppt = std::max(1, atoi(e));
    if (ks.single_pixel) ppt = 1;
    const int u = std::max(1, ks.unroll);
    g.ppt = (ppt + u - 1) / u * u;
    g.tiles_y = (num_rows + ks.tile_h * g.ppt - 1) / (ks.tile_h * g.ppt);
    g.nwg = (long)g.tiles_x * g.tiles_y;
    g.tiles_magic = tile_division_magic(g.tiles_x, g.nwg);
    return g;
}

static LaunchGeometry clip_launch_geometry(const KernelSource &ks, int region_w, int num_rows, int frames) {
    LaunchGeometry g = launch_geometry(ks, region_w, num_rows);
    const int tile_rows = (num_rows + ks.tile_h - 1) / ks.tile_h;
    int ppt = std::min(rows_per_item(g.wg1 * std::max(frames, 1)), std::max(rows_per_item(g.wg1), tile_rows));
    if (const char *e = getenv("MMHIP_PPT")) ppt = std::max(1, atoi(e));
    if (ks.single_pixel) ppt = 1;
    const int u = std::max(1, ks.unroll);
    g.ppt = (ppt + u - 1) / u * u;
    g.tiles_y = (num_rows + ks.tile_h * g.ppt - 1) / (ks.tile_h * g.ppt);
    g.nwg = (long)g.tiles_x * g.tiles_y;
    g.tiles_magic = tile_division_magic(g.tiles_x, g.nwg);
    return g;
}

struct ClipPlan { long grid_x = 0; int max_frames = 0; };
static ClipPlan clip_plan(const LaunchGeometry &g) {
    static const int env_cap = [] {
        const char *e = getenv("MMHIP_CLIP_MAX_FRAMES");
        return e && atoi(e) > 0 ? atoi(e) : 65535;
    }();
    ClipPlan p;
    p.grid_x = (g.nwg + 7) / 8 * 8;
    const long by_items = ((1L << 23) - 1) / p.grid_x;
    p.max_frames = (int)std::min<long>(std::min(65535, env_cap), by_items);
    return p;
}

static int geometry_out(const KernelSource &ks, int region_w, int num_rows, int64_t *out, int clip_frames = 0) {
    if (region_w < 1 || num_rows < 1) return fail("launch geometry: empty region");
    const LaunchGeometry g = clip_frames > 0 ? clip_launch_geometry(ks, region_w, num_rows, clip_frames) : launch_geometry(ks, region_w, num_rows);
    int m = 0;
    for (unsigned v = (unsigned)(g.tiles_x > 1 ? g.tiles_x - 1 : 1); v; v >>= 1) ++m;
    const int64_t v[MMHIP_GEOMETRY_FIELDS] = {g.tiles_x, g.tiles_y, g.wg1, g.nwg, g.ppt, ks.tile_w, ks.tile_h, ks.unroll,
                                              ks.pair_mode, ks.single_pixel, ks.xcd_order, (int64_t)g.tiles_magic,
                                              (g.nwg >> (m + 3)) << (m + 3)};
    memcpy(out, v, sizeof v);
    return 0;
}

int mmhip_filter_launch_geometry(const mmhip_filter *f, int region_w, int num_rows, int64_t *out) {
    return geometry_out(f->ks, region_w, num_rows, out);
}

int mmhip_filter_clip_launch_geometry(const mmhip_filter *f, int region_w, int num_rows, int frames, int64_t *out) {
    if (frames < 1) return fail("clip launch geometry: num_frames must be at least 1");
    return geometry_out(f->ks, region_w, num_rows, out, frames);
}

int mmhip_filter_clip_batch_plan(const mmhip_filter *f, int region_w, int num_rows, int frames, int64_t *out) {
    if (frames < 1) return fail("clip batch plan: num_frames must be at least 1");
    if (region_w < 1 || num_rows < 1) return fail("clip batch plan: empty region");
    const bool batched = f->ks.natives.empty() && f->closures.empty();
    const ClipPlan p = clip_plan(clip_launch_geometry(f->ks, region_w, num_rows, frames));
    const int64_t per = batched ? p.max_frames : 0;
    const int64_t v[MMHIP_CLIP_PLAN_FIELDS] = {p.grid_x, per, per ? (frames + per - 1) / per : 0, !f->ks.prologue_uses_time};
    memcpy(out, v, sizeof v);
    return 0;
}

int mmhip_filter_num_closures(const mmhip_filter *f) { return (int)f->closures.size(); }

int mmhip_filter_closure_launch_geometry(const mmhip_filter *f, int closure, int width, int height, int64_t *out) {
    if (closure < 0 || closure >= (int)f->closures.size()) return fail("launch geometry: no such closure image");
    return geometry_out(f->closures[closure].ks, width, height, out);
}

static int grow_launch_buffers(LaunchBuffers &b, const KernelSource &ks, int region_w, int num_rows, bool rows, hipStream_t s) {
    auto wait = [s] { return hipStreamSynchronize(s); };
    HIP_TRY(b.xtab.grow((size_t)region_w * sizeof(float), wait));
    HIP_TRY(b.ytab.grow((size_t)num_rows * sizeof(float), wait));
    if (rows) HIP_TRY(b.rowtab.grow((size_t)ks.row_values * num_rows * sizeof(float), wait));
    HIP_TRY(b.xy.grow(std::max(ks.xy_bytes, 256), wait, true));
    return 0;
}

struct RecordedCall { size_t k; HNativeRec rec; const std::string *func; };
static int recorded_calls(const KernelSource &ks, const char *host, std::vector<RecordedCall> *calls) {
    calls->clear();
    if (ks.natives.empty()) return 0;
    int ctr[4];
    memcpy(ctr, host + ks.native_ctr_offset, sizeof ctr);
    if (ctr[2])
        return fail("native filters are called more than " + std::to_string((int)MM_NATIVE_DYN_CALLS) +
                    " times from inside a loop of the frame-constant code: not supported");
    for (size_t k = 0; k < ks.natives.size(); ++k) {
        RecordedCall c;
        c.k = k;
        memcpy(&c.rec, host + ks.natives[k].record_offset, sizeof c.rec);
        if (!c.rec.executed) continue;
        if (c.rec.index < 0 || c.rec.index >= ks.native_sites) return fail("internal: native call record names no call site");
        c.func = &ks.natives[c.rec.index].func;
        calls->push_back(c);
    }
    std::sort(calls->begin(), calls->end(), [](const RecordedCall &x, const RecordedCall &y) { return x.rec.pad < y.rec.pad; });
    return 0;
}

static bool same_native_call(const RecordedCall &c, const RecordedCall &m, const std::vector<int> &alias, int closure_slot_base) {
    if (*c.func != *m.func || c.rec.nargs != m.rec.nargs) return false;
    for (int i = 0; i < c.rec.nargs && i < 4; ++i) {
        const HNativeArg &x = c.rec.args[i], &y = m.rec.args[i];
        if (x.kind != y.kind) return false;
        if (x.kind != 2) {
            if (x.i != y.i || memcmp(&x.f, &y.f, sizeof x.f) != 0) return false;
            continue;
        }
        int idx = x.img.idx;
        const int rel = idx - closure_slot_base;
        if (rel >= 0 && rel < (int)alias.size()) {
            if (alias[rel] < 0) return false;
            idx = alias[rel];
        }
        if (idx != y.img.idx || x.img.pw != y.img.pw || x.img.ph != y.img.ph || x.img.resized != y.img.resized ||
            memcmp(&x.img.xf, &y.img.xf, sizeof x.img.xf) != 0 || memcmp(&x.img.yf, &y.img.yf, sizeof x.img.yf) != 0)
            return false;
    }
    return true;
}

static int render_closure(mmhip_invocation *inv, mmhip_filter *f, int cid, const HArgs &main_args, hipStream_t s,
                          const std::vector<RecordedCall> &main_done) {
    mmhip_closure_kernel &ck = f->closures[cid];
    auto &st = inv->closure_state[cid];
    const int w = main_args.render_width, h = main_args.render_height;
    if (st.map && (st.w != w || st.h != h)) {
        HIP_TRY(hipDeviceSynchronize());
        st.map.reset();
        for (DeviceBuffer &m : st.native_results) m.reset();
    }
    if (!st.map) {
        HIP_TRY(st.map.grow((size_t)w * h * 16));
        st.w = w;
        st.h = h;
    }
    if (grow_launch_buffers(st.launch, ck.ks, w, h, false, s) != 0) return -1;
    HArgs a = main_args;
    a.region_x = a.region_y = 0;
    a.region_width = w;
    a.region_height = h;
    a.sampling_offset_x = a.sampling_offset_y = 0.0f;
    a.first_row = 0;
    a.num_rows = h;
    a.output_bpp = 4;
    a.row_stride = w * 4;
    a.floatmap = 1;
    a.out = st.map.get();
    a.xtab = st.launch.xtab.get<float>();
    a.ytab = st.launch.ytab.get<float>();
    const LaunchGeometry geo = launch_geometry(ck.ks, w, h);
    a.ppt = geo.ppt;
    a.tiles_magic = geo.tiles_magic;
    char *xy = st.launch.xy.get<char>();
    void *params[] = {&a, &xy};
    const int n = std::max(w, h);
    a.native_slot_base = st.native_slot_base;
    HIP_TRY(hipModuleLaunchKernel(ck.f_pro, (unsigned)((n + 255) / 256), 1, 1, 256, 1, 1, 0, s, params, nullptr));
    if (!ck.ks.natives.empty()) {
        std::vector<char> host(ck.ks.xy_bytes);
        HIP_TRY(hipMemcpyAsync(host.data(), xy, host.size(), hipMemcpyDeviceToHost, s));
        HIP_TRY(hipStreamSynchronize(s));
        std::vector<RecordedCall> calls;
        if (recorded_calls(ck.ks, host.data(), &calls) != 0) return -1;
        std::vector<int> alias(ck.ks.natives.size(), -1);
        for (const RecordedCall &call : calls) {
            const size_t k = call.k;
            const HNativeRec &rec = call.rec;
            bool aliased = false;
            for (const RecordedCall &m : main_done) {
                const int mslot = inv->native_slot_base + (int)m.k;
                const NativeEntry &me = inv->natives[m.k];
                if (!same_native_call(call, m, alias, st.native_slot_base) || !me.map || inv->images[mslot].kind != IMG_FLOATMAP ||
                    inv->images[mslot].w != w || inv->images[mslot].h != h || me.rows.first > 0 || me.rows.second < h)
                    continue;
                inv->images[st.native_slot_base + (int)k] = inv->images[mslot];
                alias[k] = mslot;
                aliased = true;
                break;
            }
            if (aliased) continue;
            for (int i = 0; i < rec.nargs && i < 4; ++i)
                if (rec.args[i].kind == 2 && rec.args[i].img.idx <= -2)
                    return fail("a filter closure rendered for a native filter hands another closure to a native filter: not supported");
            HIP_TRY(st.native_results[k].grow((size_t)w * h * 16));
            std::string err;
            int lo = 0, hi = h;
            if (run_native_filter(*call.func, rec, inv->images, w, h, st.native_results[k].get<float>(), inv->ws, s, &err, &lo, &hi) != 0)
                return fail(err);
            inv->images[st.native_slot_base + (int)k] = floatmap_desc(st.native_results[k].get(), w, h);
        }
        if (upload_image_table(inv, s) != 0) return -1;
    }
    HIP_TRY(hipModuleLaunchKernel(ck.f_pix, (unsigned)geo.nwg, 1, 1, 256, 1, 1, 0, s, params, nullptr));
    return 0;
}

static bool direct_output_wanted(const mmhip_filter *f, const HArgs &a) {
    return f->ks.direct_native >= 0 && !a.floatmap && a.output_bpp == 4 && (a.row_stride & 3) == 0 && ((uintptr_t)a.out & 3) == 0 &&
           !getenv("MMHIP_NO_DIRECT_NATIVE");
}

static bool samples_own_pixels(const HArgs &a, const std::vector<float> &xt, const std::vector<float> &yt) {
    const HImageDesc m = floatmap_desc(nullptr, a.render_width, a.render_height);
    for (int c = 0; c < a.region_width; ++c)
        if (lrintf(m.ax * xt[c] + m.bx) != (long)a.region_x + c) return false;
    for (int r = 0; r < a.num_rows; ++r)
        if (lrintf(m.ay * yt[r] + m.by) != (long)a.first_row + r) return false;
    return true;
}

static int direct_output(const mmhip_filter *f, const HArgs &a, hipStream_t s, NativeDirectOut *direct) {
    const bool try_direct = direct_output_wanted(f, a);
    std::vector<float> xt, yt;
    if (try_direct) {
        xt.resize(a.region_width);
        yt.resize(a.num_rows);
        HIP_TRY(hipMemcpyAsync(xt.data(), a.xtab, xt.size() * sizeof(float), hipMemcpyDeviceToHost, s));
        HIP_TRY(hipMemcpyAsync(yt.data(), a.ytab, yt.size() * sizeof(float), hipMemcpyDeviceToHost, s));
    }
    HIP_TRY(hipStreamSynchronize(s));
    if (!try_direct) return 0;
    if (!samples_own_pixels(a, xt, yt)) return 0;
    direct->out = a.out;
    direct->row_stride = a.row_stride;
    direct->first_row = a.first_row;
    direct->num_rows = a.num_rows;
    direct->region_x = a.region_x;
    direct->region_w = a.region_width;
    return 0;
}

static int render_closure_args(mmhip_invocation *inv, mmhip_filter *f, const HArgs &a, hipStream_t s,
                               const std::vector<RecordedCall> &done, HNativeRec &rec, std::vector<HImageDesc> &images_k) {
    for (int i = 0; i < rec.nargs && i < 4; ++i) {
        HImage &img = rec.args[i].img;
        if (rec.args[i].kind != 2 || img.idx > -2) continue;
        const int cid = -2 - img.idx;
        if (cid >= (int)f->closures.size()) return fail("internal: closure image without a render kernel");
        if (render_closure(inv, f, cid, a, s, done) != 0) return -1;
        if (images_k.empty()) images_k = inv->images;
        img.idx = (int)images_k.size();
        img.pw = a.render_width;
        img.ph = a.render_height;
        img.xf = img.yf = 1.0f;
        img.resized = 0;
        images_k.push_back(floatmap_desc(inv->closure_state[cid].map.get(), a.render_width, a.render_height));
    }
    return 0;
}

enum { NO_FRAME_KEY = INT32_MIN };
static int view_sequence_args(const mmhip_invocation *inv, int frame, const std::string &func, const HNativeRec &rec,
                              std::vector<HImageDesc> &images_k, int *frame_key) {
    *frame_key = NO_FRAME_KEY;
    if (inv->native_input_frame != MMHIP_NATIVE_FRAME_CURRENT) return 0;
    for (int i = 0; i < rec.nargs && i < 4; ++i) {
        const int idx = rec.args[i].img.idx;
        if (rec.args[i].kind != 2 || idx < 0 || idx >= inv->native_slot_base) continue;
        const HImageDesc &d = inv->images[idx];
        if (d.kind != IMG_DRAWABLE || d.num_frames <= 1) continue;
        if (frame < 0 || frame >= d.num_frames)
            return fail((func == "RENDER" ? std::string("render()") : func.rfind("native_filter_", 0) == 0 ? func.substr(14) : func) + ": frame " + std::to_string(frame) + " is outside the input sequence (" + std::to_string(d.num_frames) +
                        " frames; native input frame mode `current')");
        if (images_k.empty()) images_k = inv->images;
        HImageDesc &v = images_k[idx];
        v.data = (const char *)d.data + (size_t)frame * d.w * d.h * 4;
        v.num_frames = 1;
        *frame_key = frame;
    }
    return 0;
}

static bool memo_hit(const mmhip_invocation *inv, const NativeEntry &e, const HNativeRec &rec, int frame_key, int want_lo, int want_hi,
                     std::vector<unsigned long long> *deps) {
    for (int i = 0; i < rec.nargs && i < 4; ++i)
        if (rec.args[i].kind == 2 && rec.args[i].img.idx >= inv->native_slot_base &&
            rec.args[i].img.idx < inv->native_slot_base + (int)inv->natives.size())
            deps->push_back(inv->natives[rec.args[i].img.idx - inv->native_slot_base].gen);
    return e.map && e.memo_gen == inv->input_generation && e.memo_frame == frame_key && memcmp(&e.memo, &rec, sizeof rec) == 0 && e.memo_deps == *deps &&
           e.rows.first <= want_lo && e.rows.second >= want_hi;
}

static void drop_native_map(mmhip_invocation *inv, size_t k, bool *table_changed) {
    NativeEntry &e = inv->natives[k];
    e.map.reset();
    e.memo_gen = e.seen_gen = ~0ULL;
    e.rows = {0, 0};
    HImageDesc &d = inv->images[inv->native_slot_base + (int)k];
    d.kind = IMG_NULL;
    d.data = nullptr;
    *table_changed = true;
}

static int run_natives(mmhip_invocation *inv, mmhip_filter *f, const HArgs &a, hipStream_t s, bool *direct_written) {
    std::vector<char> host(f->ks.xy_bytes);
    HIP_TRY(hipMemcpyAsync(host.data(), inv->launch.xy.get(), host.size(), hipMemcpyDeviceToHost, s));
    NativeDirectOut direct;
    if (direct_output(f, a, s, &direct) != 0) return -1;
    inv->ws.env.supersampling = f->kopt.supersampling;
    inv->ws.env.edge_x = f->kopt.edge_x;
    inv->ws.env.edge_y = f->kopt.edge_y;
    inv->ws.env.edge_color_x = inv->edge_color_x;
    inv->ws.env.edge_color_y = inv->edge_color_y;
    inv->ws.gauss_tolerance = f->opts.gauss_mode == MMHIP_GAUSS_TOLERANCE;
    int want_lo = 0, want_hi = a.render_height;
    if (inv->native_row_margin >= 0 && a.region_x == 0 && a.region_y == 0 && a.region_width == a.render_width &&
        a.region_height == a.render_height) {
        want_lo = std::max(0, a.first_row - inv->native_row_margin);
        want_hi = std::min(a.render_height, a.first_row + a.num_rows + inv->native_row_margin);
    }
    const bool whole = a.region_x == 0 && a.region_y == 0 && a.region_width == a.render_width &&
                       a.region_height == a.render_height && a.first_row == 0 && a.num_rows == a.render_height;
    bool table_changed = false;
    std::vector<RecordedCall> calls, done;
    if (recorded_calls(f->ks, host.data(), &calls) != 0) return -1;
    for (const RecordedCall &call : calls) {
        const size_t k = call.k;
        NativeEntry &e = inv->natives[k];
        HNativeRec rec = call.rec;
        if (e.map && (e.w != a.render_width || e.h != a.render_height)) {
            HIP_TRY(hipDeviceSynchronize());
            drop_native_map(inv, k, &table_changed);
        }
        std::vector<HImageDesc> images_k;
        if (render_closure_args(inv, f, a, s, done, rec, images_k) != 0) return -1;
        const bool closure_args = !images_k.empty();
        int frame_key = NO_FRAME_KEY;
        if (view_sequence_args(inv, a.frame, *call.func, rec, images_k, &frame_key) != 0) return -1;
        std::vector<unsigned long long> deps;
        if (memo_hit(inv, e, rec, frame_key, want_lo, want_hi, &deps) && !closure_args) {
            done.push_back(call);
            continue;
        }
        HIP_TRY(e.map.grow((size_t)a.render_width * a.render_height * 16));
        e.w = a.render_width;
        e.h = a.render_height;
        std::string err;
        int got_lo = want_lo, got_hi = want_hi;
        NativeDirectOut *dk = (direct.out && (int)k == f->ks.direct_native) ? &direct : nullptr;
        if (dk) {
            dk->skip_map = whole && !(e.seen_gen == inv->input_generation && e.seen_frame == frame_key && e.memo_deps == deps &&
                                      memcmp(&e.seen, &rec, sizeof rec) == 0);
            e.seen = rec;
            e.seen_frame = frame_key;
            e.seen_gen = inv->input_generation;
        }
        if (run_native_filter(*call.func, rec, images_k.empty() ? inv->images : images_k, a.render_width, a.render_height,
                              e.map.get<float>(), inv->ws, s, &err, &got_lo, &got_hi, dk) != 0)
            return fail(err);
        e.gen = ++inv->native_gen_counter;
        e.memo_deps = deps;
        if (dk && dk->written) *direct_written = true;
        if (dk && dk->written && dk->tolerance) ++inv->tolerance_blur_launches;
        if (dk && dk->written && dk->skip_map) {
            e.memo_gen = ~0ULL;
            e.rows = {0, 0};
            continue;
        }
        inv->images[inv->native_slot_base + (int)k] = floatmap_desc(e.map.get(), a.render_width, a.render_height);
        e.memo = rec;
        e.memo_frame = frame_key;
        e.memo_gen = inv->input_generation;
        e.rows = {got_lo, got_hi};
        table_changed = true;
        done.push_back(call);
    }
    if (f->ks.native_sites < (int)f->ks.natives.size()) {
        std::vector<char> used(f->ks.natives.size(), 0);
        for (const RecordedCall &call : calls) used[call.k] = 1;
        for (size_t k = (size_t)f->ks.native_sites; k < f->ks.natives.size(); ++k) {
            if (used[k] || !inv->natives[k].map) continue;
            HIP_TRY(hipStreamSynchronize(s));
            drop_native_map(inv, k, &table_changed);
        }
    }
    if (table_changed && upload_image_table(inv, s) != 0) return -1;
    return 0;
}

static void bake_uservals(Block &b, const std::map<int, Primary> &consts) {
    for (Stmt *st : b) {
        if (st->kind == Stmt::Assign && st->rhs.kind == Rhs::Op && st->rhs.args.size() == 1 &&
            st->rhs.args[0].kind == Primary::IntConst) {
            const char *n = st->rhs.op->cname;
            if (!strcmp(n, "USERVAL_INT_ACCESS") || !strcmp(n, "USERVAL_FLOAT_ACCESS") || !strcmp(n, "USERVAL_BOOL_ACCESS")) {
                auto it = consts.find(st->rhs.args[0].i);
                if (it != consts.end()) st->rhs = Rhs::P(it->second);
            }
        }
        if (st->kind == Stmt::If) { bake_uservals(st->then_, consts); bake_uservals(st->else_, consts); }
        if (st->kind == Stmt::While) bake_uservals(st->body, consts);
    }
}

static mmhip_filter *compile_ir_specialized(const mmhip_filter *f, const std::map<int, Primary> &consts, bool peel = true) {
    mmhip_filter *sp = mmhip_filter_new_empty();
    try {
        sp->code.reset(new FilterCode());
        load_ir_json(sp->module, *sp->code, (f->ir_json_raw.empty() ? f->ir_json : f->ir_json_raw).c_str());
        bake_uservals(sp->code->body, consts);
        specialize_constants(*sp->code);
        const bool peeled = peel && pair_peel_enabled() && peel_first_trips(*sp->code);
        for (auto &sub : sp->code->closure_renders) {
            bake_uservals(sub->body, consts);
            specialize_constants(*sub);
        }
        std::string err;
        if (!mmhip_filter_finalize(sp, f->kopt, &err)) throw CompileError(err);
        if (peeled && !sp->ks.pair_exit) {
            mmhip_filter_free(sp);
            return compile_ir_specialized(f, consts, false);
        }
        sp->opts = f->opts;
        sp->opts.specialize_uservals = 0;
    } catch (const std::exception &e) {
        g_err = e.what();
        mmhip_filter_free(sp);
        return nullptr;
    }
    return sp;
}

extern "C" mmhip_filter *mmhip_filter_specialized(const mmhip_filter *f, int n, const int *indices, const double *values) {
    std::map<int, Primary> consts;
    const auto &uvs = f->module.main->uservals;
    for (int i = 0; i < n; ++i) {
        if (indices[i] < 0 || indices[i] >= (int)uvs.size()) { g_err = "user value index out of range"; return nullptr; }
        const UservalInfo &u = uvs[indices[i]];
        if (u.kind == UvKind::Float) consts[u.index] = Primary::F((float)values[i]);
        else if (u.kind == UvKind::Int || u.kind == UvKind::Bool) consts[u.index] = Primary::I((int)values[i]);
    }
    mmhip_options o = f->opts;
    o.specialize_uservals = 0;
    return f->source.empty() ? compile_ir_specialized(f, consts) : compile_source(f->source.c_str(), &o, &consts);
}

static mmhip_filter *active_filter(mmhip_invocation *inv, int frame = 0, float t = 0.0f) {
    mmhip_filter *f = inv->f;
    if (!f->specialize || !f->ks.natives.empty() || (f->source.empty() && f->ir_json.empty() && f->ir_json_raw.empty())) return f;
    g_err.clear();
    const auto &uvs = f->module.main->uservals;
    std::string key;
    std::map<int, Primary> consts;
    for (const UservalInfo &u : uvs) {
        if (u.kind == UvKind::Int || u.kind == UvKind::Bool) consts[u.index] = Primary::I(inv->uv[u.index].i);
        else if (u.kind == UvKind::Float) consts[u.index] = Primary::F(inv->uv[u.index].f);
        else continue;
        key.append((const char *)&inv->uv[u.index], sizeof(HUserval));
    }
    if (consts.empty()) return f;
    auto it = f->spec_cache.find(key);
    if (it != f->spec_cache.end()) return it->second ? it->second : f;
    if (f->spec_min_uses > 1) {
        if (f->spec_uses.size() > 1024) f->spec_uses.clear();
        auto &u = f->spec_uses[key];
        if (u.count == 0 || u.frame != frame || u.t != t) {
            ++u.count;
            u.frame = frame;
            u.t = t;
        }
        if (u.count < f->spec_min_uses) return f;
    }
    f->spec_uses.erase(key);
    mmhip_options o = f->opts;
    o.specialize_uservals = 0;
    mmhip_filter *sp = f->source.empty() ? compile_ir_specialized(f, consts) : compile_source(f->source.c_str(), &o, &consts);
    if (sp && mmhip_filter_jit(sp, 1) < 0) { mmhip_filter_free(sp); sp = nullptr; }
    f->spec_cache[key] = sp;
    return sp ? sp : f;
}

static HArgs render_args(const mmhip_invocation *inv, int frame, float t, int region_x, int region_y, int region_w, int region_h,
                         int first_row, int last_row, void *out_device, int row_stride, int bpp, int floatmap) {
    HArgs a{};
    a.img_width = inv->img_w;
    a.img_height = inv->img_h;
    a.render_width = inv->render_w;
    a.render_height = inv->render_h;
    a.frame_render_width = inv->render_w;
    a.frame_render_height = inv->render_h;
    a.t = t;
    a.frame = frame;
    a.R = (float)sqrt(2.0);
    a.region_x = region_x;
    a.region_y = region_y;
    a.region_width = region_w;
    a.region_height = region_h;
    a.sampling_offset_x = inv->sampling_offset_x;
    a.sampling_offset_y = inv->sampling_offset_y;
    a.first_row = first_row;
    a.num_rows = last_row - first_row;
    a.output_bpp = bpp;
    a.row_stride = row_stride;
    a.floatmap = floatmap;
    a.edge_color_x = inv->edge_color_x;
    a.edge_color_y = inv->edge_color_y;
    a.uservals = inv->d_uv.get<HUserval>();
    a.images = inv->d_images.get<HImageDesc>();
    a.num_images = (uint32_t)inv->images.size();
    a.curves = inv->d_curves.get();
    a.gradients = inv->d_gradients.get();
    a.out = out_device;
    a.native_slot_base = inv->native_slot_base;
    return a;
}

int mmhip_render(mmhip_invocation *inv, int frame, float t, int region_x, int region_y, int region_w, int region_h,
                 int first_row, int last_row, void *out_device, int row_stride, int bpp, int floatmap, void *stream) {
    mmhip_filter *f = active_filter(inv, frame, t);
    hipStream_t s = stream ? (hipStream_t)stream : inv->stream;
    if (bpp < 1 || bpp > 4) return fail("output_bpp must be 1..4");
    if (region_w <= 0 || region_h <= 0) return fail("empty region");
    if (first_row < 0) first_row = 0;
    if (last_row > region_y + region_h) last_row = region_y + region_h;
    if (last_row <= first_row) return 0;
    if (upload_tables(inv, s) != 0) return -1;

    HArgs a = render_args(inv, frame, t, region_x, region_y, region_w, region_h, first_row, last_row, out_device, row_stride, bpp, floatmap);
    const size_t rowtab_bytes = inv->launch.rowtab.bytes;
    if (grow_launch_buffers(inv->launch, f->ks, region_w, a.num_rows, f->ks.row_values > 0, s) != 0) return -1;
    if (inv->launch.rowtab.bytes != rowtab_bytes) inv->pro_filter = nullptr;
    a.xtab = inv->launch.xtab.get<float>();
    a.ytab = inv->launch.ytab.get<float>();
    if (f->ks.row_values > 0) a.rowtab = inv->launch.rowtab.get<float>();
    char *xy = inv->launch.xy.get<char>();
    void *params[] = {&a, &xy};
    bool direct_written = false;
    {
        HArgs key = a;
        key.out = nullptr;
        key.row_stride = key.output_bpp = key.floatmap = key.ppt = 0;
        key.tiles_magic = 0;
        if (!f->ks.prologue_uses_time) { key.t = 0.0f; key.frame = 0; }
        const bool fresh = f->ks.natives.empty() && inv->pro_filter == f && inv->pro_stream == (void *)s &&
                           inv->pro_generation == inv->table_generation &&
                           memcmp(&key, &inv->pro_args, sizeof key) == 0;
        if (!fresh) {
            int n = std::max(region_w, a.num_rows);
            HIP_TRY(hipModuleLaunchKernel(f->f_pro, (unsigned)((n + 255) / 256), 1, 1, 256, 1, 1, 0, s, params, nullptr));
            if (f->ks.row_values > 0)
                HIP_TRY(hipModuleLaunchKernel(f->f_rows, (unsigned)((a.num_rows + 255) / 256), 1, 1, 256, 1, 1, 0, s, params, nullptr));
            if (!f->ks.natives.empty() && run_natives(inv, f, a, s, &direct_written) != 0) return -1;
            inv->pro_args = key;
            inv->pro_filter = f;
            inv->pro_stream = (void *)s;
            inv->pro_generation = inv->table_generation;
        }
    }
    const LaunchGeometry geo = launch_geometry(f->ks, region_w, a.num_rows);
    const long nwg = geo.nwg;
    if (nwg > 0x7fffffffL) return fail("region too large for one launch");
    a.ppt = geo.ppt;
    a.tiles_magic = geo.tiles_magic;
    if (inv->timing) {
        if (next_event_pair(inv) != 0) return -1;
        HIP_TRY(hipEventRecord(inv->ev0, s));
    }
    if (direct_written) ++inv->direct_native_launches;
    if (!direct_written) HIP_TRY(hipModuleLaunchKernel(f->f_pix, (unsigned)nwg, 1, 1, 256, 1, 1, 0, s, params, nullptr));
    if (inv->timing) {
        HIP_TRY(hipEventRecord(inv->ev1, s));
        inv->ev_valid = true;
    }
    return 0;
}

long mmhip_clip_batched_launches(mmhip_invocation *inv) { return inv->clip_batched_launches; }
long mmhip_clip_prologue_frames(mmhip_invocation *inv) { return inv->clip_prologue_frames; }
long mmhip_clip_native_batches(mmhip_invocation *inv) { return inv->clip_native_batches; }
long mmhip_clip_native_blurs(mmhip_invocation *inv) { return inv->clip_native_blurs; }
long mmhip_clip_native_direct_frames(mmhip_invocation *inv) { return inv->clip_native_direct_frames; }

struct HClipFrame { float t; int frame; };
struct HClip { const HClipFrame *frames; long long frame_stride; int xy_stride; int rowtab_stride; int nwg; int images_stride; };
static_assert(sizeof(HClip) == 32, "mm_clip layout");

static bool clip_native_eligible(const mmhip_filter *f, int native_row_margin) {
    if (f->ks.natives.empty() || f->ks.native_sites != (int)f->ks.natives.size() || !f->closures.empty()) return false;
    for (const NativeCall &nc : f->ks.natives)
        if (nc.func != "native_filter_gaussian_blur") return false;
    const char *seg = getenv("MMHIP_GAUSS_SEGMENTS");
    return f->opts.gauss_mode == MMHIP_GAUSS_EXACT && !(seg && *seg) && native_row_margin < 0;
}

struct ClipNativePlan { bool eligible = false; int per_batch = 0; size_t bytes_per_frame = 0; };
static ClipNativePlan clip_native_plan(const mmhip_filter *f, int native_row_margin, const ClipPlan &plan, int render_w, int render_h) {
    static const size_t budget = [] {
        const char *e = getenv("MMHIP_CLIP_NATIVE_BYTES");
        const long long v = e ? atoll(e) : 0;
        return v > 0 ? (size_t)v : (size_t)8 << 30;
    }();
    ClipNativePlan p;
    p.eligible = clip_native_eligible(f, native_row_margin);
    if (!p.eligible || render_w < 1 || render_h < 1) return p;
    size_t ck = 0, map = 0;
    gaussian_blur_batch_job_bytes(render_w, render_h, &ck, &map);
    p.bytes_per_frame = (size_t)f->ks.native_sites * (ck + 2 * map);
    const size_t by_bytes = budget / p.bytes_per_frame;
    const int per = (int)std::min<size_t>(std::min(plan.max_frames, 65535), by_bytes);
    p.per_batch = per < 2 ? 0 : per;
    return p;
}

int mmhip_filter_clip_native_plan(const mmhip_filter *f, int region_w, int num_rows, int render_w, int render_h, int frames, int64_t *out) {
    if (frames < 1) return fail("clip native plan: num_frames must be at least 1");
    if (region_w < 1 || num_rows < 1 || render_w < 1 || render_h < 1) return fail("clip native plan: empty region");
    const ClipPlan cp = clip_plan(clip_launch_geometry(f->ks, region_w, num_rows, frames));
    const ClipNativePlan p = clip_native_plan(f, -1, cp, render_w, render_h);
    const int64_t v[MMHIP_CLIP_NATIVE_PLAN_FIELDS] = {p.eligible, p.per_batch, p.per_batch ? (frames + p.per_batch - 1) / p.per_batch : 0,
                                                      (int64_t)p.bytes_per_frame};
    memcpy(out, v, sizeof v);
    return 0;
}

struct ClipCall {
    mmhip_invocation *inv;
    mmhip_filter *f;
    hipStream_t s;
    HArgs a;
    HClip c;
    char *xy;
    LaunchGeometry geo;
    ClipPlan plan;
    bool per_frame, rows;
    size_t xy_stride;
    int64_t frame_stride;
    const int *frames;
    const float *ts;
    void *stream_arg;
    std::vector<char> records;
    int direct_ok = -1;
};

static int clip_native_batch(ClipCall &cc, int b0, int n) {
    mmhip_invocation *inv = cc.inv;
    mmhip_filter *f = cc.f;
    hipStream_t s = cc.s;
    const KernelSource &ks = f->ks;
    HArgs a = cc.a;
    HClip c = cc.c;
    char *xy = cc.xy;
    a.out = (char *)cc.a.out + (int64_t)b0 * cc.frame_stride;
    c.frames = cc.c.frames + b0;
    c.images_stride = 0;
    void *params[] = {&a, &xy, &c};
    const int num_rows = a.num_rows, region_w = a.region_width;
    const unsigned pro_x = (unsigned)((std::max(region_w, num_rows) + 255) / 256), rows_x = (unsigned)((num_rows + 255) / 256);
    const unsigned pro_frames = cc.per_frame ? (unsigned)n : b0 == 0 ? 1u : 0u;
    if (pro_frames) {
        HIP_TRY(hipModuleLaunchKernel(f->f_pro_clip, pro_x, pro_frames, 1, 256, 1, 1, 0, s, params, nullptr));
        if (cc.rows) HIP_TRY(hipModuleLaunchKernel(f->f_rows_clip, rows_x, pro_frames, 1, 256, 1, 1, 0, s, params, nullptr));
        cc.records.resize(cc.xy_stride * pro_frames);
        HIP_TRY(hipMemcpyAsync(cc.records.data(), xy, cc.records.size(), hipMemcpyDeviceToHost, s));
    }
    std::vector<float> xt, yt;
    const bool ask_direct = cc.direct_ok < 0 && direct_output_wanted(f, a) && (cc.frame_stride & 3) == 0;
    if (ask_direct) {
        xt.resize(region_w);
        yt.resize(num_rows);
        HIP_TRY(hipMemcpyAsync(xt.data(), a.xtab, xt.size() * sizeof(float), hipMemcpyDeviceToHost, s));
        HIP_TRY(hipMemcpyAsync(yt.data(), a.ytab, yt.size() * sizeof(float), hipMemcpyDeviceToHost, s));
    }
    HIP_TRY(hipStreamSynchronize(s));
    if (cc.direct_ok < 0) cc.direct_ok = ask_direct && samples_own_pixels(a, xt, yt) ? 1 : 0;
    auto frame_by_frame = [&]() -> int {
        for (int i = b0; i < b0 + n; ++i)
            if (mmhip_render(inv, cc.frames[i], cc.ts[i], a.region_x, a.region_y, a.region_width, a.region_height, a.first_row,
                             a.first_row + a.num_rows, (char *)cc.a.out + (int64_t)i * cc.frame_stride, a.row_stride, a.output_bpp, a.floatmap,
                             cc.stream_arg) != 0)
                return -1;
        return 0;
    };

    struct Comp { size_t k; HNativeRec rec; int frame; std::vector<HImageDesc> view; float *map = nullptr; };
    const int sites = ks.native_sites, base = inv->native_slot_base;
    std::vector<Comp> comps;
    std::vector<int> of_frame((size_t)n * sites, -1);
    std::map<std::string, int> known;
    std::vector<char> is_dep;
    std::vector<RecordedCall> calls;
    for (int i = 0; i < n; ++i) {
        if (recorded_calls(ks, cc.records.data() + (cc.per_frame ? (size_t)i * cc.xy_stride : 0), &calls) != 0) return -1;
        size_t last_k = 0;
        for (size_t q = 0; q < calls.size(); ++q) {
            const RecordedCall &call = calls[q];
            if (q > 0 && call.k <= last_k) return frame_by_frame();
            last_k = call.k;
            std::string key((const char *)&call.k, sizeof call.k);
            key.append((const char *)&call.rec, sizeof call.rec);
            for (int j = 0; j < call.rec.nargs && j < 4; ++j) {
                const HNativeArg &arg = call.rec.args[j];
                if (arg.kind != 2 || arg.img.idx < base || arg.img.idx >= base + sites) continue;
                const int dep = of_frame[(size_t)i * sites + (arg.img.idx - base)];
                key.append((const char *)&dep, sizeof dep);
                if (dep >= 0) is_dep[dep] = 1;
            }
            std::vector<HImageDesc> view;
            int frame_key = NO_FRAME_KEY;
            if (view_sequence_args(inv, cc.frames[b0 + i], *call.func, call.rec, view, &frame_key) != 0) return -1;
            key.append((const char *)&frame_key, sizeof frame_key);
            auto it = known.find(key);
            if (it == known.end()) {
                it = known.emplace(key, (int)comps.size()).first;
                comps.push_back(Comp{call.k, call.rec, i, std::move(view)});
                is_dep.push_back(0);
            }
            of_frame[(size_t)i * sites + call.k] = it->second;
        }
    }
    bool direct = cc.direct_ok == 1 && ((uintptr_t)a.out & 3) == 0;
    if (direct) {
        std::vector<char> taken(comps.size(), 0);
        for (int i = 0; i < n && direct; ++i) {
            const int id = of_frame[(size_t)i * sites + ks.direct_native];
            direct = id >= 0 && !taken[id] && !is_dep[id];
            if (direct) taken[id] = 1;
        }
    }
    size_t ck_bytes = 0, map_bytes = 0;
    gaussian_blur_batch_job_bytes(a.render_width, a.render_height, &ck_bytes, &map_bytes);
    std::vector<size_t> per_site(sites, 0);
    size_t kept = 0;
    for (const Comp &cp : comps) {
        ++per_site[cp.k];
        if (!(direct && (int)cp.k == ks.direct_native)) ++kept;
    }
    const size_t jobs_max = comps.empty() ? 0 : *std::max_element(per_site.begin(), per_site.end());
    const size_t images_n = inv->images.size();
    const size_t images_bytes = ((size_t)n * images_n * sizeof(HImageDesc) + 255) & ~(size_t)255;
    const size_t tables_bytes = images_bytes + gaussian_blur_batch_table_bytes(comps.size());
    ClipNativeBuffers &nb = inv->clip_native;
    auto idle = [] { return hipSuccess; };
    HIP_TRY(nb.work.grow(jobs_max * (ck_bytes + map_bytes), idle));
    HIP_TRY(nb.maps.grow(kept * map_bytes, idle));
    HIP_TRY(nb.tables.grow(tables_bytes, idle));
    if (nb.uploaded_pending) HIP_TRY(hipEventSynchronize(nb.uploaded));
    nb.uploaded_pending = false;
    HIP_TRY(nb.host.grow(tables_bytes));
    {
        size_t m = 0;
        for (Comp &cp : comps)
            if (!(direct && (int)cp.k == ks.direct_native)) cp.map = (float *)(nb.maps.get<char>() + (m++) * map_bytes);
    }
    HImageDesc *tables = (HImageDesc *)nb.host.p;
    HImageDesc null_desc{};
    null_desc.kind = IMG_NULL;
    for (int i = 0; i < n; ++i) {
        HImageDesc *t = tables + (size_t)i * images_n;
        std::copy(inv->images.begin(), inv->images.end(), t);
        for (int k = 0; k < sites; ++k) {
            const int id = of_frame[(size_t)i * sites + k];
            t[base + k] = id >= 0 && comps[id].map ? floatmap_desc(comps[id].map, a.render_width, a.render_height) : null_desc;
        }
    }
    inv->ws.env.supersampling = f->kopt.supersampling;
    inv->ws.env.edge_x = f->kopt.edge_x;
    inv->ws.env.edge_y = f->kopt.edge_y;
    inv->ws.env.edge_color_x = inv->edge_color_x;
    inv->ws.env.edge_color_y = inv->edge_color_y;
    inv->ws.gauss_tolerance = false;
    for (const Comp &cp : comps) {
        const int idx = cp.rec.args[0].img.idx;
        const HImageDesc *t = cp.view.empty() ? tables + (size_t)cp.frame * images_n : cp.view.data();
        const bool own_result = idx >= base && idx < base + sites && of_frame[(size_t)cp.frame * sites + (idx - base)] >= 0 && (size_t)(idx - base) < cp.k;
        const bool bound_input = idx >= 0 && idx < base;
        if (!(own_result || bound_input) ||
            !gaussian_blur_batchable(cp.rec, t, (int)images_n, a.render_width, a.render_height, inv->ws.env, nullptr, nullptr))
            return frame_by_frame();
    }
    NativeDirectOut dout;
    dout.row_stride = a.row_stride;
    dout.first_row = a.first_row;
    dout.num_rows = a.num_rows;
    dout.region_x = a.region_x;
    dout.region_w = a.region_width;
    std::vector<std::vector<GaussClipGroup>> groups(sites);
    std::vector<GaussClipLaunch> launches(sites);
    size_t at = images_bytes;
    std::string err;
    for (int k = 0; k < sites; ++k) {
        std::vector<GaussClipJob> jobs;
        const bool packs = direct && k == ks.direct_native;
        for (size_t id = 0; id < comps.size(); ++id) {
            const Comp &cp = comps[id];
            if ((int)cp.k != k) continue;
            char *w = nb.work.get<char>() + jobs.size() * (ck_bytes + map_bytes);
            jobs.push_back(GaussClipJob{cp.rec, cp.view.empty() ? tables + (size_t)cp.frame * images_n : cp.view.data(), (int)images_n, (double *)w, (float *)(w + ck_bytes), cp.map,
                                        packs ? (unsigned char *)a.out + (int64_t)cp.frame * cc.frame_stride : nullptr});
        }
        launches[k].render_w = a.render_width;
        launches[k].render_h = a.render_height;
        launches[k].direct = packs ? &dout : nullptr;
        launches[k].write_map = !packs;
        if (jobs.empty()) continue;
        if (gaussian_blur_batch_tables(jobs, launches[k], inv->ws.env, (char *)nb.host.p + at, nb.tables.get<char>() + at, &groups[k], &err) != 0)
            return fail(err);
        at += gaussian_blur_batch_table_bytes(jobs.size());
    }
    if (!nb.uploaded) HIP_TRY(hipEventCreateWithFlags(&nb.uploaded, hipEventDisableTiming));
    HIP_TRY(hipMemcpyAsync(nb.tables.get(), nb.host.p, tables_bytes, hipMemcpyHostToDevice, s));
    HIP_TRY(hipEventRecord(nb.uploaded, s));
    nb.uploaded_pending = true;
    for (int k = 0; k < sites; ++k)
        if (!groups[k].empty() && gaussian_blur_batch_launch(groups[k], launches[k], inv->ws, s, &err) != 0) return fail(err);
    ++inv->clip_native_batches;
    inv->clip_native_blurs += (long)comps.size();
    if (direct) {
        inv->clip_native_direct_frames += n;
        return 0;
    }
    a.images = nb.tables.get<HImageDesc>();
    c.images_stride = (int)images_n;
    if (inv->timing) {
        if (next_event_pair(inv) != 0) return -1;
        HIP_TRY(hipEventRecord(inv->ev0, s));
    }
    HIP_TRY(hipModuleLaunchKernel(f->f_pix_clip, (unsigned)cc.plan.grid_x, (unsigned)n, 1, 256, 1, 1, 0, s, params, nullptr));
    if (inv->timing) {
        HIP_TRY(hipEventRecord(inv->ev1, s));
        inv->ev_valid = true;
    }
    return 0;
}

int mmhip_render_clip(mmhip_invocation *inv, int num_frames, const int *frames, const float *ts, int region_x, int region_y,
                      int region_w, int region_h, int first_row, int last_row, void *out_device, int row_stride,
                      int64_t frame_stride, int bpp, int floatmap, void *stream) {
    if (num_frames < 1) return fail("render_clip: num_frames must be at least 1");
    if (!frames || !ts) return fail("render_clip: frames and ts must be arrays of num_frames entries");
    if (bpp < 1 || bpp > 4) return fail("output_bpp must be 1..4");
    if (region_w <= 0 || region_h <= 0) return fail("empty region");
    if (first_row < 0) first_row = 0;
    if (last_row > region_y + region_h) last_row = region_y + region_h;
    if (last_row <= first_row) return 0;
    const int num_rows = last_row - first_row;
    const int64_t band = floatmap ? (int64_t)num_rows * 16 * inv->render_w
                                  : (int64_t)(num_rows - 1) * row_stride + (int64_t)region_w * bpp;
    if (frame_stride < band)
        return fail("render_clip: frame_stride " + std::to_string(frame_stride) + " is smaller than one frame's band (" +
                    std::to_string(band) + " bytes)");
    mmhip_filter *f = active_filter(inv, frames[0], ts[0]);
    hipStream_t s = stream ? (hipStream_t)stream : inv->stream;
    const LaunchGeometry geo = clip_launch_geometry(f->ks, region_w, num_rows, num_frames);
    const ClipPlan plan = clip_plan(geo);
    const bool natives = !f->ks.natives.empty();
    const ClipNativePlan nplan = natives ? clip_native_plan(f, inv->native_row_margin, plan, inv->render_w, inv->render_h) : ClipNativePlan();
    if ((natives && nplan.per_batch < 1) || !f->closures.empty() || plan.max_frames < 1) {
        for (int i = 0; i < num_frames; ++i)
            if (mmhip_render(inv, frames[i], ts[i], region_x, region_y, region_w, region_h, first_row, last_row,
                             (char *)out_device + (int64_t)i * frame_stride, row_stride, bpp, floatmap, stream) != 0)
                return -1;
        return 0;
    }
    if (mmhip_filter_jit_clip(f, 1) < 0) return -1;
    if (upload_tables(inv, s) != 0) return -1;

    HArgs a = render_args(inv, frames[0], ts[0], region_x, region_y, region_w, region_h, first_row, last_row, out_device, row_stride, bpp, floatmap);
    const bool per_frame = f->ks.prologue_uses_time;
    const bool rows = f->ks.row_values > 0;
    const int per_batch = std::min(num_frames, natives ? nplan.per_batch : plan.max_frames);
    const size_t xy_stride = ((size_t)std::max(f->ks.xy_bytes, 256) + 255) / 256 * 256;
    const size_t rowtab_stride = (size_t)f->ks.row_values * num_rows;
    const int slots = per_frame ? per_batch : 1;
    if (rowtab_stride * slots > (size_t)INT32_MAX || xy_stride * slots > (size_t)INT32_MAX)
        return fail("render_clip: the batch's row tables are too large; lower MMHIP_CLIP_MAX_FRAMES");
    if (grow_launch_buffers(inv->launch, f->ks, region_w, num_rows, false, s) != 0) return -1;
    inv->pro_filter = nullptr;
    auto wait = [s] { return hipStreamSynchronize(s); };
    HIP_TRY(inv->clip.xy.grow(xy_stride * slots, wait, true));
    if (rows) HIP_TRY(inv->clip.rowtab.grow(rowtab_stride * slots * sizeof(float), wait));
    ClipBuffers::Table &tab = inv->clip.table[inv->clip.next_table++ & 1];
    if (tab.pending) HIP_TRY(hipEventSynchronize(tab.uploaded));
    tab.pending = false;
    const size_t tab_bytes = (size_t)num_frames * sizeof(HClipFrame);
    HIP_TRY(tab.host.grow(tab_bytes));
    HIP_TRY(tab.dev.grow(tab_bytes, wait));
    if (!tab.uploaded) HIP_TRY(hipEventCreateWithFlags(&tab.uploaded, hipEventDisableTiming));
    HClipFrame *hf = (HClipFrame *)tab.host.p;
    for (int i = 0; i < num_frames; ++i) hf[i] = HClipFrame{ts[i], frames[i]};
    HIP_TRY(hipMemcpyAsync(tab.dev.get(), hf, tab_bytes, hipMemcpyHostToDevice, s));
    HIP_TRY(hipEventRecord(tab.uploaded, s));
    tab.pending = true;

    a.xtab = inv->launch.xtab.get<float>();
    a.ytab = inv->launch.ytab.get<float>();
    if (rows) a.rowtab = inv->clip.rowtab.get<float>();
    a.ppt = geo.ppt;
    a.tiles_magic = geo.tiles_magic;
    char *xy = inv->clip.xy.get<char>();
    HClip c{};
    c.frame_stride = frame_stride;
    c.xy_stride = per_frame ? (int)xy_stride : 0;
    c.rowtab_stride = per_frame ? (int)rowtab_stride : 0;
    c.nwg = (int)geo.nwg;
    if (natives) {
        ClipCall cc{inv, f, s, a, c, xy, geo, plan, per_frame, rows, xy_stride, frame_stride, frames, ts, stream, {}, -1};
        cc.c.frames = tab.dev.get<HClipFrame>();
        for (int b0 = 0; b0 < num_frames; b0 += per_batch)
            if (clip_native_batch(cc, b0, std::min(per_batch, num_frames - b0)) != 0) return -1;
        return 0;
    }
    void *params[] = {&a, &xy, &c};
    const unsigned pro_x = (unsigned)((std::max(region_w, num_rows) + 255) / 256), rows_x = (unsigned)((num_rows + 255) / 256);
    for (int b0 = 0; b0 < num_frames; b0 += per_batch) {
        const int n = std::min(per_batch, num_frames - b0);
        a.out = (char *)out_device + (int64_t)b0 * frame_stride;
        c.frames = tab.dev.get<HClipFrame>() + b0;
        const unsigned pro_frames = per_frame ? (unsigned)n : b0 == 0 ? 1u : 0u;
        if (pro_frames) {
            HIP_TRY(hipModuleLaunchKernel(f->f_pro_clip, pro_x, pro_frames, 1, 256, 1, 1, 0, s, params, nullptr));
            if (rows) HIP_TRY(hipModuleLaunchKernel(f->f_rows_clip, rows_x, pro_frames, 1, 256, 1, 1, 0, s, params, nullptr));
            inv->clip_prologue_frames += pro_frames;
        }
        if (inv->timing) {
            if (next_event_pair(inv) != 0) return -1;
            HIP_TRY(hipEventRecord(inv->ev0, s));
        }
        HIP_TRY(hipModuleLaunchKernel(f->f_pix_clip, (unsigned)plan.grid_x, (unsigned)n, 1, 256, 1, 1, 0, s, params, nullptr));
        ++inv->clip_batched_launches;
        if (inv->timing) {
            HIP_TRY(hipEventRecord(inv->ev1, s));
            inv->ev_valid = true;
        }
    }
    return 0;
}

int mmhip_render_supersampled(mmhip_invocation *inv, int frame, float t, int region_x, int region_y, int region_w,
                              int region_h, void *out_device, int row_stride, int bpp, void *stream) {
    hipStream_t s = stream ? (hipStream_t)stream : inv->stream;
    const size_t long_bytes = (size_t)(region_w + 1) * bpp * region_h;
    const size_t short_bytes = (size_t)region_w * bpp * region_h;
    if (inv->ss_lines.grow(long_bytes + short_bytes, hipDeviceSynchronize) != hipSuccess)
        return fail("out of device memory for the supersampling lines");
    unsigned char *tmp = inv->ss_lines.get<unsigned char>();
    const float ox = inv->sampling_offset_x, oy = inv->sampling_offset_y;
    inv->sampling_offset_x = -0.5f;
    inv->sampling_offset_y = -0.5f;
    int rc = mmhip_render(inv, frame, t, region_x, region_y, region_w + 1, region_h, region_y, region_y + region_h, tmp,
                          (region_w + 1) * bpp, bpp, 0, s);
    inv->sampling_offset_x = 0.f;
    inv->sampling_offset_y = 0.f;
    if (rc == 0)
        rc = mmhip_render(inv, frame, t, region_x, region_y, region_w, region_h, region_y, region_y + region_h,
                          tmp + long_bytes, region_w * bpp, bpp, 0, s);
    inv->sampling_offset_x = ox;
    inv->sampling_offset_y = oy;
    if (rc != 0) return rc;
    launch_supersample_combine(tmp, tmp + long_bytes, (unsigned char *)out_device, region_w, region_h, bpp, row_stride, s);
    return 0;
}

struct ClipSsPlan { int per_batch = 0; size_t bytes_per_frame = 0, long_pitch = 0; };
static ClipSsPlan clip_ss_plan(const mmhip_filter *f, bool host_between, int region_w, int region_h, int bpp, int frames) {
    static const size_t budget = [] {
// ... 17 lines not shown
    return p;
}

int mmhip_filter_clip_supersample_plan(const mmhip_filter *f, int region_w, int region_h, int bpp, int frames, int64_t *out) {
    if (frames < 1) return fail("clip supersample plan: num_frames must be at least 1");
    if (bpp < 1 || bpp > 4) return fail("output_bpp must be 1..4");
    if (region_w < 1 || region_h < 1) return fail("clip supersample plan: empty region");
    const ClipSsPlan p = clip_ss_plan(f, !f->ks.natives.empty() || !f->closures.empty(), region_w, region_h, bpp, frames);
    const int64_t v[MMHIP_CLIP_SS_PLAN_FIELDS] = {p.per_batch > 0, p.per_batch, p.per_batch ? (frames + p.per_batch - 1) / p.per_batch : 0,
                                                  (int64_t)p.bytes_per_frame, (int64_t)p.long_pitch, SS_CLIP_ROWS, SS_CLIP_PIXELS};
    memcpy(out, v, sizeof v);
    return 0;
}

long mmhip_clip_supersampled_batches(mmhip_invocation *inv) { return inv->clip_supersampled_batches; }

struct SamplingOffsetGuard {
    mmhip_invocation *inv;
    float ox, oy;
    explicit SamplingOffsetGuard(mmhip_invocation *i) : inv(i), ox(i->sampling_offset_x), oy(i->sampling_offset_y) {}
    ~SamplingOffsetGuard() { inv->sampling_offset_x = ox; inv->sampling_offset_y = oy; }
    void set(float v) { inv->sampling_offset_x = inv->sampling_offset_y = v; }
};

int mmhip_render_clip_supersampled(mmhip_invocation *inv, int num_frames, const int *frames, const float *ts, int region_x,
                                   int region_y, int region_w, int region_h, void *out_device, int row_stride,
                                   int64_t frame_stride, int bpp, void *stream) {
    if (num_frames < 1) return fail("render_clip_supersampled: num_frames must be at least 1");
    if (!frames || !ts) return fail("render_clip_supersampled: frames and ts must be arrays of num_frames entries");
    if (bpp < 1 || bpp > 4) return fail("output_bpp must be 1..4");
    if (region_w <= 0 || region_h <= 0) return fail("empty region");
    const int64_t band = (int64_t)(region_h - 1) * row_stride + (int64_t)region_w * bpp;
    if (frame_stride < band)
        return fail("render_clip_supersampled: frame_stride " + std::to_string(frame_stride) + " is smaller than one frame's band (" +
                    std::to_string(band) + " bytes)");
    const bool host_between = !inv->f->ks.natives.empty() || !inv->f->closures.empty();
    const ClipSsPlan plan = clip_ss_plan(host_between ? inv->f : active_filter(inv, frames[0], ts[0]), host_between, region_w,
                                         region_h, bpp, num_frames);
    if (plan.per_batch < 1) {
        for (int i = 0; i < num_frames; ++i)
            if (mmhip_render_supersampled(inv, frames[i], ts[i], region_x, region_y, region_w, region_h,
                                          (char *)out_device + (int64_t)i * frame_stride, row_stride, bpp, stream) != 0)
                return -1;
        return 0;
    }
    hipStream_t s = stream ? (hipStream_t)stream : inv->stream;
    const int per_batch = plan.per_batch;
    const size_t long_frame = (size_t)region_h * plan.long_pitch, short_frame = (size_t)region_h * region_w * bpp;
    if (inv->clip_ss.grow((size_t)per_batch * plan.bytes_per_frame, hipDeviceSynchronize) != hipSuccess)
        return fail("out of device memory for the supersampling slices of a clip; lower MMHIP_CLIP_SS_BYTES");
    unsigned char *longs = inv->clip_ss.get<unsigned char>(), *shorts = longs + (size_t)per_batch * long_frame;
    SamplingOffsetGuard offsets(inv);
    for (int b0 = 0; b0 < num_frames; b0 += per_batch) {
        const int n = std::min(per_batch, num_frames - b0);
        offsets.set(-0.5f);
        if (mmhip_render_clip(inv, n, frames + b0, ts + b0, region_x, region_y, region_w + 1, region_h, region_y, region_y + region_h,
                              longs, (int)plan.long_pitch, (int64_t)long_frame, bpp, 0, s) != 0)
            return -1;
        offsets.set(0.f);
        if (mmhip_render_clip(inv, n, frames + b0, ts + b0, region_x, region_y, region_w, region_h, region_y, region_y + region_h,
                              shorts, region_w * bpp, (int64_t)short_frame, bpp, 0, s) != 0)
            return -1;
        std::string err;
        if (launch_supersample_combine_clip(longs, shorts, (unsigned char *)out_device + (int64_t)b0 * frame_stride, region_w, region_h,
                                            bpp, row_stride, frame_stride, n, inv->ws, s, &err) != 0)
            return fail(err);
        ++inv->clip_supersampled_batches;
    }
    return 0;
}

int mmhip_sync(mmhip_invocation *inv) {
    HIP_TRY(hipStreamSynchronize(inv->stream));
    return 0;
}

int mmhip_render_host(mmhip_invocation *inv, int frame, float t, uint8_t *out_rgba) {
    size_t bytes = (size_t)inv->render_w * inv->render_h * 4;
    void *d = nullptr;
    HIP_TRY(hipMalloc(&d, bytes));
    int rc = mmhip_render(inv, frame, t, 0, 0, inv->render_w, inv->render_h, 0, inv->render_h, d, inv->render_w * 4, 4, 0,
                          nullptr);
    if (rc == 0) {
        hipError_t e = hipStreamSynchronize(inv->stream);
        if (e == hipSuccess) e = hipMemcpy(out_rgba, d, bytes, hipMemcpyDeviceToHost);
        if (e != hipSuccess) rc = fail(std::string("render: ") + hipGetErrorString(e));
    }
    (void)hipFree(d);
    return rc;
}

void *mmhip_device_alloc(size_t bytes) {
    void *p = nullptr;
    if (hipMalloc(&p, bytes) != hipSuccess) { fail("hipMalloc failed"); return nullptr; }
    return p;
}
void mmhip_device_free(void *p) { (void)hipFree(p); }
int mmhip_copy_to_host(void *dst, const void *src, size_t bytes) {
    HIP_TRY(hipMemcpy(dst, src, bytes, hipMemcpyDeviceToHost));
    return 0;
}
int mmhip_copy_to_device(void *dst, const void *src, size_t bytes) {
    HIP_TRY(hipMemcpy(dst, src, bytes, hipMemcpyHostToDevice));
    return 0;
}
int mmhip_set_device(int ordinal) {
    HIP_TRY(hipSetDevice(ordinal));
    return 0;
}
int mmhip_device_count(void) {
    int n = 0;
    if (hipGetDeviceCount(&n) != hipSuccess) return 0;
    return n;
}

}
```

### mathmap_amd/csrc/runtime_internal.h

```cpp
#pragma once
#include <hip/hip_runtime.h>

#include <map>
#include <memory>
#include <string>
#include <utility>
#include <vector>

#include "../../include/mmhip.h"
#include "front.h"
#include "hipgen.h"
#include "mm_host_abi.h"
#include "native_filters.h"

namespace mm { void load_ir_json(Module &mod, FilterCode &code, const char *json); }

struct mmhip_closure_kernel {
    mm::KernelSource ks;
    std::vector<char> code_object;
    hipModule_t mod = nullptr;
    hipFunction_t f_pro = nullptr, f_pix = nullptr;
    bool loaded = false;
};

struct mmhip_filter {
    std::vector<mmhip_closure_kernel> closures;
    mm::Module module;
    std::unique_ptr<mm::FilterCode> code;
    mm::KernelOptions kopt;
    mm::KernelSource ks;
    std::string ir_json;
    std::string ir_json_raw;
    std::vector<char> code_object;
    hipModule_t mod = nullptr;
    hipFunction_t f_pro = nullptr, f_pix = nullptr;
    hipFunction_t f_rows = nullptr;
    bool loaded = false;
    double jit_seconds = 0;
    mm::KernelSource clip_ks;
    std::vector<char> clip_code_object;
    hipModule_t clip_mod = nullptr;
    hipFunction_t f_pro_clip = nullptr, f_rows_clip = nullptr, f_pix_clip = nullptr;
    bool clip_loaded = false;
    std::string source;
    mmhip_options opts{};
    bool specialize = false;
    std::map<std::string, mmhip_filter *> spec_cache;
    struct SpecUse { int count = 0; int frame = 0; float t = 0.0f; };
    std::map<std::string, SpecUse> spec_uses;
    int spec_min_uses = 1;
};

struct DeviceBuffer {
    void *p = nullptr;
    size_t bytes = 0;
    DeviceBuffer() = default;
    DeviceBuffer(DeviceBuffer &&o) noexcept : p(std::exchange(o.p, nullptr)), bytes(std::exchange(o.bytes, 0)) {}
    DeviceBuffer &operator=(DeviceBuffer &&o) noexcept {
        if (this != &o) { reset(); p = std::exchange(o.p, nullptr); bytes = std::exchange(o.bytes, 0); }
        return *this;
    }
    ~DeviceBuffer() { reset(); }
    void reset() { if (p) (void)hipFree(p); p = nullptr; bytes = 0; }
    template <class T = void> T *get() const { return (T *)p; }
    explicit operator bool() const { return p != nullptr; }
    static hipError_t no_wait() { return hipSuccess; }
    template <class Wait = hipError_t (*)()> hipError_t grow(size_t need, Wait wait = no_wait, bool zero = false) {
        if (need <= bytes) return hipSuccess;
        if (p) {
            const hipError_t e = wait();
            if (e != hipSuccess) return e;
            reset();
        }
        hipError_t e = hipMalloc(&p, need);
        if (e != hipSuccess) { p = nullptr; return e; }
        bytes = need;
        if (zero && (e = hipMemset(p, 0, need)) != hipSuccess) reset();
        return e;
    }
};

struct LaunchBuffers { DeviceBuffer xy, xtab, ytab, rowtab; };

struct PinnedBuffer {
    void *p = nullptr;
    size_t bytes = 0;
    PinnedBuffer() = default;
    PinnedBuffer(const PinnedBuffer &) = delete;
    PinnedBuffer &operator=(const PinnedBuffer &) = delete;
    ~PinnedBuffer() { if (p) (void)hipHostFree(p); }
    hipError_t grow(size_t need) {
        if (need <= bytes) return hipSuccess;
        if (p) (void)hipHostFree(p);
        p = nullptr;
        bytes = 0;
        const hipError_t e = hipHostMalloc(&p, need, hipHostMallocDefault);
        if (e != hipSuccess) { p = nullptr; return e; }
        bytes = need;
        return hipSuccess;
    }
};

struct ClipBuffers {
    DeviceBuffer xy, rowtab;
    struct Table {
        PinnedBuffer host;
        DeviceBuffer dev;
        hipEvent_t uploaded = nullptr;
        bool pending = false;
        ~Table() { if (uploaded) (void)hipEventDestroy(uploaded); }
    } table[2];
    unsigned next_table = 0;
};

struct ClipNativeBuffers {
    DeviceBuffer work, maps, tables;
    PinnedBuffer host;
    hipEvent_t uploaded = nullptr;
    bool uploaded_pending = false;
    ~ClipNativeBuffers() { if (uploaded) (void)hipEventDestroy(uploaded); }
};

struct NativeEntry {
    DeviceBuffer map;
    int w = 0, h = 0;
    unsigned long long gen = 0;
    mm::HNativeRec memo{};
    int memo_frame = 0, seen_frame = 0;
    unsigned long long memo_gen = 0;
    std::vector<unsigned long long> memo_deps;
    mm::HNativeRec seen{};
    unsigned long long seen_gen = ~0ULL;
    std::pair<int, int> rows{0, 0};
};

struct OwnedStream {
    hipStream_t s = nullptr;
    OwnedStream() = default;
    OwnedStream(const OwnedStream &) = delete;
    ~OwnedStream() { if (s) (void)hipStreamDestroy(s); }
    operator hipStream_t() const { return s; }
};

struct mmhip_invocation {
    ~mmhip_invocation();
    OwnedStream stream;
    mmhip_filter *f = nullptr;
    int img_w = 0, img_h = 0, render_w = 0, render_h = 0;
    std::vector<mm::HUserval> uv;
    std::vector<mm::HImageDesc> images;
    std::vector<int> image_slot_of_uv;
    std::vector<float> curves;
    std::vector<uint32_t> gradients;
    DeviceBuffer d_uv, d_images, d_curves, d_gradients;
    int native_slot_base = 0;
    bool tables_dirty = true;
    std::vector<DeviceBuffer> owned;
    std::vector<NativeEntry> natives;
    unsigned long long native_gen_counter = 0;
    struct ClosureState {
        DeviceBuffer map;
        int w = 0, h = 0;
        LaunchBuffers launch;
        int native_slot_base = 0;
        std::vector<DeviceBuffer> native_results;
    };
    std::vector<ClosureState> closure_state;
    DeviceBuffer ss_lines;
    int native_row_margin = -1;
    int native_input_frame = 0;
    long direct_native_launches = 0;
    long tolerance_blur_launches = 0;
    mm::HArgs pro_args{};
    const mmhip_filter *pro_filter = nullptr;
    void *pro_stream = nullptr;
    unsigned long long pro_generation = 0, table_generation = 1;
    unsigned long long input_generation = 1;
    LaunchBuffers launch;
    ClipBuffers clip;
    long clip_batched_launches = 0;
    long clip_prologue_frames = 0;
    ClipNativeBuffers clip_native;
    long clip_native_batches = 0;
    long clip_native_blurs = 0;
    long clip_native_direct_frames = 0;
    DeviceBuffer clip_ss;
    long clip_supersampled_batches = 0;
    uint32_t edge_color_x = 0, edge_color_y = 0;
    float sampling_offset_x = 0.f, sampling_offset_y = 0.f;
    bool timing = false;
    hipEvent_t ev0 = nullptr, ev1 = nullptr;
    bool ev_valid = false;
    std::vector<std::pair<hipEvent_t, hipEvent_t>> ev_pool;
    size_t ev_used = 0;
    mm::NativeWorkspace ws;
};


extern thread_local std::string g_mmhip_err;

mmhip_filter *mmhip_filter_new_empty();
bool mmhip_filter_finalize(mmhip_filter *f, const mm::KernelOptions &ko, std::string *err);
bool mmhip_check_options(const mmhip_options *opts);

void mmhip_unbind_image(mmhip_invocation *inv, const void *data);
```

Before: 426,700.

## Upload parameter tables through a pinned ring and cache prologue readbacks

Replaces the synchronous per-table hipMemcpy uploads, which blocked the stream, with a four-slot ring of pinned host buffers. Each slot holds all tables in one device allocation and is filled with a single async copy, guarded by events. The prologue freshness key now ignores table pointers, uses time only when hoisted code computes with it, and tracks image input generations so the device-to-host prologue readback can be skipped when records are still valid. It also adds host-wait and prologue-launch counters; in exchange it brings more bookkeeping and the risk of stale records if the freshness checks are wrong.

```diff
diff --git a/include/mmhip.h b/include/mmhip.h
--- a/include/mmhip.h
+++ b/include/mmhip.h
@@ -57,6 +57,8 @@
 const char *mmhip_filter_kernel_source(mmhip_filter *f);
 int mmhip_filter_gauss_mode(const mmhip_filter *f);
 int mmhip_filter_num_native_calls(const mmhip_filter *f);
+int mmhip_filter_prologue_reads_images(const mmhip_filter *f);
+int mmhip_filter_prologue_computes_with_time(const mmhip_filter *f);
 int mmhip_filter_builtin_ids(const mmhip_filter *f, char *buf, int cap);
 enum { MMHIP_GEOMETRY_FIELDS = 13 };
 int mmhip_filter_launch_geometry(const mmhip_filter *f, int region_w, int num_rows, int64_t *out);
@@ -121,6 +123,8 @@
 int mmhip_drain_native_kernel_ms(mmhip_invocation *inv, char *names, double *out_ms, int cap);
 long mmhip_direct_native_launches(mmhip_invocation *inv);
 long mmhip_tolerance_blur_launches(mmhip_invocation *inv);
+long mmhip_render_host_waits(mmhip_invocation *inv);
+long mmhip_prologue_launches(mmhip_invocation *inv);
 
 void *mmhip_device_alloc(size_t bytes);
 void mmhip_device_free(void *p);
diff --git a/mathmap_amd/_lib.py b/mathmap_amd/_lib.py
--- a/mathmap_amd/_lib.py
+++ b/mathmap_amd/_lib.py
@@ -59,6 +59,10 @@
     "mmhip_drain_kernel_ms": (C.c_int, [C.c_void_p, C.c_void_p, C.c_int]),
     "mmhip_direct_native_launches": (C.c_long, [C.c_void_p]),
     "mmhip_tolerance_blur_launches": (C.c_long, [C.c_void_p]),
+    "mmhip_render_host_waits": (C.c_long, [C.c_void_p]),
+    "mmhip_prologue_launches": (C.c_long, [C.c_void_p]),
+    "mmhip_filter_prologue_reads_images": (C.c_int, [C.c_void_p]),
+    "mmhip_filter_prologue_computes_with_time": (C.c_int, [C.c_void_p]),
     "mmhip_drain_native_kernel_ms": (C.c_int, [C.c_void_p, C.c_char_p, C.c_void_p, C.c_int]),
     "mmhip_set_curve": (C.c_int, [C.c_void_p, C.c_int, C.c_void_p]),
     "mmhip_set_gradient": (C.c_int, [C.c_void_p, C.c_int, C.c_void_p]),
diff --git a/mathmap_amd/api.py b/mathmap_amd/api.py
--- a/mathmap_amd/api.py
+++ b/mathmap_amd/api.py
@@ -132,6 +132,14 @@
         return {v: k for k, v in GAUSS_MODES.items()}[mode]
 
     @property
+    def prologue_reads_images(self):
+        return bool(lib().mmhip_filter_prologue_reads_images(self._h))
+
+    @property
+    def prologue_computes_with_time(self):
+        return bool(lib().mmhip_filter_prologue_computes_with_time(self._h))
+
+    @property
     def num_native_calls(self):
         return lib().mmhip_filter_num_native_calls(self._h)
 
@@ -324,6 +332,14 @@
 
     def tolerance_blur_launches(self):
         return lib().mmhip_tolerance_blur_launches(self._h)
+
+    @property
+    def render_host_waits(self):
+        return lib().mmhip_render_host_waits(self._h)
+
+    @property
+    def prologue_launches(self):
+        return lib().mmhip_prologue_launches(self._h)
 
     def render(self, t=0.0, frame=0):
         out = np.empty((self.render_height, self.render_width, 4), dtype=np.uint8)
diff --git a/mathmap_amd/csrc/hipgen.cpp b/mathmap_amd/csrc/hipgen.cpp
--- a/mathmap_amd/csrc/hipgen.cpp
+++ b/mathmap_amd/csrc/hipgen.cpp
@@ -401,6 +401,35 @@
         });
         return uses;
     }
+    static bool hoisted_computes_with_time(const Block &b) {
+        std::set<const Value *> time;
+        each_stmt(b, [&](const Stmt *s) {
+            if (s->hoisted && s->kind == Stmt::Assign && s->rhs.kind == Rhs::Internal && (s->rhs.internal == "t" || s->rhs.internal == "frame")) time.insert(s->lhs);
+            return true;
+        });
+        auto reads = [&](const Rhs &r) {
+            if (r.kind == Rhs::Prim && r.prim.kind == Primary::Val && time.count(r.prim.value)) return true;
+            for (const Primary &p : r.args)
+                if (p.kind == Primary::Val && time.count(p.value)) return true;
+            return false;
+        };
+        std::function<bool(const Block &)> uses = [&](const Block &blk) {
+            for (const Stmt *s : blk) {
+                if (s->hoisted && (reads(s->rhs) || reads(s->rhs2) || reads(s->cond))) return true;
+                if (uses(s->then_) || uses(s->else_) || uses(s->phis) || uses(s->body)) return true;
+            }
+            return false;
+        };
+        return uses(b);
+    }
+    static bool hoisted_reads_images(const Block &b) {
+        bool reads = false;
+        each_stmt(b, [&](const Stmt *s) {
+            reads = reads || ((s->hoisted || s->in_row) && (is_op(s, "ORIG_VAL") || (s->kind == Stmt::Assign && s->rhs.kind == Rhs::FilterCall)));
+            return true;
+        });
+        return reads;
+    }
     static void pixel_stats(const Block &b, int &stmts, int &fetches) {
         each_stmt(b, [&](const Stmt *s) { stmts += s->in_pixel; fetches += s->in_pixel && is_op(s, "ORIG_VAL"); return s->in_pixel; });
     }
@@ -852,6 +881,8 @@
 
     void emit_prologue_kernel() {
         ks.prologue_uses_time = hoisted_uses_time(code.body);
+        ks.prologue_reads_images = hoisted_reads_images(code.body);
+        ks.prologue_computes_with_time = ks.prologue_uses_time && hoisted_computes_with_time(code.body);
         ks.prologue_name = "mm_prologue";
         ks.pixel_name = "mm_pixels";
         auto tables = [](const std::string &first) {
diff --git a/mathmap_amd/csrc/hipgen.h b/mathmap_amd/csrc/hipgen.h
--- a/mathmap_amd/csrc/hipgen.h
+++ b/mathmap_amd/csrc/hipgen.h
@@ -38,6 +38,8 @@
     int tile_w = 16, tile_h = 16;
     int unroll = 1;
     bool prologue_uses_time = true;
+    bool prologue_computes_with_time = true;
+    bool prologue_reads_images = false;
     bool single_pixel = false;
     bool pair_mode = false;
     bool pair_exit = false;
diff --git a/mathmap_amd/csrc/native_filters.h b/mathmap_amd/csrc/native_filters.h
--- a/mathmap_amd/csrc/native_filters.h
+++ b/mathmap_amd/csrc/native_filters.h
@@ -19,6 +19,7 @@
     bool gauss_tolerance = false;
     void *scratch = nullptr;
     size_t scratch_bytes = 0;
+    long host_waits = 0;
     bool keep_tolerance_map = false;
     void *reserve(size_t bytes);
     void release();
diff --git a/mathmap_amd/csrc/native_filters.hip b/mathmap_amd/csrc/native_filters.hip
--- a/mathmap_amd/csrc/native_filters.hip
+++ b/mathmap_amd/csrc/native_filters.hip
@@ -777,6 +777,7 @@
         int *flags = (int *)aux;
         float *d_curve = (float *)(aux + (size_t)std::max(w, h) * 4 * sizeof(int));
         float *d_sum = d_curve + curve.size();
+        ++ws.host_waits;
         if (hipMemcpyAsync(d_curve, curve.data(), curve.size() * 4, hipMemcpyHostToDevice, s) != hipSuccess ||
             hipMemcpyAsync(d_sum, sum.data(), sum.size() * 4, hipMemcpyHostToDevice, s) != hipSuccess ||
             hipStreamSynchronize(s) != hipSuccess) {
diff --git a/mathmap_amd/csrc/runtime.cpp b/mathmap_amd/csrc/runtime.cpp
--- a/mathmap_amd/csrc/runtime.cpp
+++ b/mathmap_amd/csrc/runtime.cpp
@@ -210,6 +210,8 @@
 const char *mmhip_filter_kernel_source(mmhip_filter *f) { return f->ks.source.c_str(); }
 int mmhip_filter_gauss_mode(const mmhip_filter *f) { return f->opts.gauss_mode; }
 int mmhip_filter_num_native_calls(const mmhip_filter *f) { return f->ks.native_sites; }
+int mmhip_filter_prologue_reads_images(const mmhip_filter *f) { return f->ks.prologue_reads_images ? 1 : 0; }
+int mmhip_filter_prologue_computes_with_time(const mmhip_filter *f) { return f->ks.prologue_computes_with_time ? 1 : 0; }
 
 int mmhip_filter_builtin_ids(const mmhip_filter *f, char *buf, int cap) {
     std::string s;
@@ -396,10 +398,17 @@
     };
     hipError_t e;
     if ((e = hipStreamCreate(&inv->stream.s)) != hipSuccess) return bail("hipStreamCreate", e);
-    if ((e = inv->d_uv.grow(inv->uv.size() * sizeof(HUserval))) != hipSuccess) return bail("hipMalloc", e);
-    if ((e = inv->d_images.grow(inv->images.size() * sizeof(HImageDesc))) != hipSuccess) return bail("hipMalloc", e);
-    if ((e = inv->d_curves.grow(inv->curves.size() * 4)) != hipSuccess) return bail("hipMalloc", e);
-    if ((e = inv->d_gradients.grow(inv->gradients.size() * 4)) != hipSuccess) return bail("hipMalloc", e);
+    TableRing &ring = inv->tables;
+    auto round256 = [](size_t n) { return (n + 255) & ~(size_t)255; };
+    ring.off_uv = round256(inv->images.size() * sizeof(HImageDesc));
+    ring.off_curves = ring.off_uv + round256(inv->uv.size() * sizeof(HUserval));
+    ring.off_gradients = ring.off_curves + round256(inv->curves.size() * 4);
+    ring.bytes = ring.off_gradients + round256(inv->gradients.size() * 4);
+    for (TableRing::Slot &sl : ring.slot) {
+        if ((e = sl.dev.grow(ring.bytes)) != hipSuccess) return bail("hipMalloc", e);
+        if ((e = sl.host.grow(ring.bytes)) != hipSuccess) return bail("hipHostMalloc", e);
+        if ((e = hipEventCreateWithFlags(&sl.done, hipEventDisableTiming)) != hipSuccess) return bail("hipEventCreate", e);
+    }
     const int xy_bytes = std::max(f->ks.xy_bytes, 256);
     if ((e = inv->launch.xy.grow(xy_bytes, DeviceBuffer::no_wait, true)) != hipSuccess) return bail("hipMalloc", e);
     return inv.release();
@@ -515,7 +524,13 @@
     const UservalInfo *u = uv_info(inv, index, UvKind::Image);
     if (!u) return -1;
     int slot = inv->image_slot_of_uv[index];
-    fill_drawable_desc(inv->images[slot], device_rgba32, width, height, num_frames);
+    HImageDesc d = inv->images[slot];
+    fill_drawable_desc(d, device_rgba32, width, height, num_frames);
+    if (memcmp(&d, &inv->images[slot], sizeof d) == 0) {
+        ++inv->input_generation;
+        return 0;
+    }
+    inv->images[slot] = d;
     input_changed(inv);
     return 0;
 }
@@ -662,6 +677,8 @@
 }
 
 long mmhip_direct_native_launches(mmhip_invocation *inv) { return inv->direct_native_launches; }
+long mmhip_render_host_waits(mmhip_invocation *inv) { return inv->host_waits + inv->ws.host_waits; }
+long mmhip_prologue_launches(mmhip_invocation *inv) { return inv->prologue_launches; }
 long mmhip_tolerance_blur_launches(mmhip_invocation *inv) { return inv->tolerance_blur_launches; }
 
 int mmhip_drain_kernel_ms(mmhip_invocation *inv, double *out_ms, int cap) {
@@ -685,18 +702,46 @@
     return ms;
 }
 
-static int upload_image_table(mmhip_invocation *inv, hipStream_t s) {
-    HIP_TRY(hipStreamSynchronize(s));
-    HIP_TRY(hipMemcpy(inv->d_images.get(), inv->images.data(), inv->images.size() * sizeof(HImageDesc), hipMemcpyHostToDevice));
-    return 0;
+static int upload_table_slot(mmhip_invocation *inv, hipStream_t s) {
+    TableRing &r = inv->tables;
+    if (r.cur >= 0) {
+        TableRing::Slot &o = r.slot[r.cur];
+        HIP_TRY(hipEventRecord(o.done, s));
+        o.pending = true;
+    }
+    r.cur = (r.cur + 1) % TableRing::SLOTS;
+    TableRing::Slot &n = r.slot[r.cur];
+    if (n.pending) {
+        const hipError_t q = hipEventQuery(n.done);
+        if (q == hipErrorNotReady) {
+            ++inv->host_waits;
+            HIP_TRY(hipEventSynchronize(n.done));
+        } else if (q != hipSuccess) {
+            return fail(std::string("hipEventQuery: ") + hipGetErrorString(q));
+        }
+        n.pending = false;
+    }
+    char *h = (char *)n.host.p;
+    memcpy(h, inv->images.data(), inv->images.size() * sizeof(HImageDesc));
+    memcpy(h + r.off_uv, inv->uv.data(), inv->uv.size() * sizeof(HUserval));
+    if (!inv->curves.empty()) memcpy(h + r.off_curves, inv->curves.data(), inv->curves.size() * 4);
+    if (!inv->gradients.empty()) memcpy(h + r.off_gradients, inv->gradients.data(), inv->gradients.size() * 4);
+    HIP_TRY(hipMemcpyAsync(n.dev.get(), h, r.bytes, hipMemcpyHostToDevice, s));
+    return 0;
+}
+
+static void point_at_tables(const mmhip_invocation *inv, HArgs &a) {
+    const TableRing &r = inv->tables;
+    char *d = r.cur >= 0 ? r.slot[r.cur].dev.get<char>() : nullptr;
+    a.images = (const HImageDesc *)d;
+    a.uservals = (const HUserval *)(d + r.off_uv);
+    a.curves = inv->curves.empty() ? nullptr : d + r.off_curves;
+    a.gradients = inv->gradients.empty() ? nullptr : d + r.off_gradients;
 }
 
 static int upload_tables(mmhip_invocation *inv, hipStream_t s) {
     if (!inv->tables_dirty) return 0;
-    if (upload_image_table(inv, s) != 0) return -1;
-    HIP_TRY(hipMemcpy(inv->d_uv.get(), inv->uv.data(), inv->uv.size() * sizeof(HUserval), hipMemcpyHostToDevice));
-    if (inv->d_curves) HIP_TRY(hipMemcpy(inv->d_curves.get(), inv->curves.data(), inv->curves.size() * 4, hipMemcpyHostToDevice));
-    if (inv->d_gradients) HIP_TRY(hipMemcpy(inv->d_gradients.get(), inv->gradients.data(), inv->gradients.size() * 4, hipMemcpyHostToDevice));
+    if (upload_table_slot(inv, s) != 0) return -1;
     inv->tables_dirty = false;
     ++inv->table_generation;
     return 0;
@@ -793,8 +838,8 @@
     return geometry_out(f->closures[closure].ks, width, height, out);
 }
 
-static int grow_launch_buffers(LaunchBuffers &b, const KernelSource &ks, int region_w, int num_rows, bool rows, hipStream_t s) {
-    auto wait = [s] { return hipStreamSynchronize(s); };
+static int grow_launch_buffers(mmhip_invocation *inv, LaunchBuffers &b, const KernelSource &ks, int region_w, int num_rows, bool rows, hipStream_t s) {
+    auto wait = [inv, s] { ++inv->host_waits; return hipStreamSynchronize(s); };
     HIP_TRY(b.xtab.grow((size_t)region_w * sizeof(float), wait));
     HIP_TRY(b.ytab.grow((size_t)num_rows * sizeof(float), wait));
     if (rows) HIP_TRY(b.rowtab.grow((size_t)ks.row_values * num_rows * sizeof(float), wait));
@@ -846,12 +891,15 @@
     return true;
 }
 
-static int render_closure(mmhip_invocation *inv, mmhip_filter *f, int cid, const HArgs &main_args, hipStream_t s,
+static int render_closure(mmhip_invocation *inv, mmhip_filter *f, int cid, const HArgs &main_args_in, hipStream_t s,
                           const std::vector<RecordedCall> &main_done) {
     mmhip_closure_kernel &ck = f->closures[cid];
     auto &st = inv->closure_state[cid];
+    HArgs main_args = main_args_in;
+    point_at_tables(inv, main_args);
     const int w = main_args.render_width, h = main_args.render_height;
     if (st.map && (st.w != w || st.h != h)) {
+        ++inv->host_waits;
         HIP_TRY(hipDeviceSynchronize());
         st.map.reset();
         for (DeviceBuffer &m : st.native_results) m.reset();
@@ -861,7 +909,7 @@
         st.w = w;
         st.h = h;
     }
-    if (grow_launch_buffers(st.launch, ck.ks, w, h, false, s) != 0) return -1;
+    if (grow_launch_buffers(inv, st.launch, ck.ks, w, h, false, s) != 0) return -1;
     HArgs a = main_args;
     a.region_x = a.region_y = 0;
     a.region_width = w;
@@ -886,6 +934,7 @@
     if (!ck.ks.natives.empty()) {
         std::vector<char> host(ck.ks.xy_bytes);
         HIP_TRY(hipMemcpyAsync(host.data(), xy, host.size(), hipMemcpyDeviceToHost, s));
+        ++inv->host_waits;
         HIP_TRY(hipStreamSynchronize(s));
         std::vector<RecordedCall> calls;
         if (recorded_calls(ck.ks, host.data(), &calls) != 0) return -1;
@@ -916,7 +965,8 @@
                 return fail(err);
             inv->images[st.native_slot_base + (int)k] = floatmap_desc(st.native_results[k].get(), w, h);
         }
-        if (upload_image_table(inv, s) != 0) return -1;
+        if (upload_table_slot(inv, s) != 0) return -1;
+        point_at_tables(inv, a);
     }
     HIP_TRY(hipModuleLaunchKernel(ck.f_pix, (unsigned)geo.nwg, 1, 1, 256, 1, 1, 0, s, params, nullptr));
     return 0;
@@ -936,24 +986,21 @@
     return true;
 }
 
-static int direct_output(const mmhip_filter *f, const HArgs &a, hipStream_t s, NativeDirectOut *direct) {
-    const bool try_direct = direct_output_wanted(f, a);
+static int read_back_prologue(mmhip_invocation *inv, const mmhip_filter *f, const HArgs &a, hipStream_t s) {
+    inv->pro_records.resize(f->ks.xy_bytes);
+    inv->pro_own_pixels = -1;
+    HIP_TRY(hipMemcpyAsync(inv->pro_records.data(), inv->launch.xy.get(), inv->pro_records.size(), hipMemcpyDeviceToHost, s));
+    const bool ask = f->ks.direct_native >= 0;
     std::vector<float> xt, yt;
-    if (try_direct) {
+    if (ask) {
         xt.resize(a.region_width);
         yt.resize(a.num_rows);
         HIP_TRY(hipMemcpyAsync(xt.data(), a.xtab, xt.size() * sizeof(float), hipMemcpyDeviceToHost, s));
         HIP_TRY(hipMemcpyAsync(yt.data(), a.ytab, yt.size() * sizeof(float), hipMemcpyDeviceToHost, s));
     }
+    ++inv->host_waits;
     HIP_TRY(hipStreamSynchronize(s));
-    if (!try_direct) return 0;
-    if (!samples_own_pixels(a, xt, yt)) return 0;
-    direct->out = a.out;
-    direct->row_stride = a.row_stride;
-    direct->first_row = a.first_row;
-    direct->num_rows = a.num_rows;
-    direct->region_x = a.region_x;
-    direct->region_w = a.region_width;
+    if (ask) inv->pro_own_pixels = samples_own_pixels(a, xt, yt) ? 1 : 0;
     return 0;
 }
 
@@ -1019,11 +1066,18 @@
     *table_changed = true;
 }
 
-static int run_natives(mmhip_invocation *inv, mmhip_filter *f, const HArgs &a, hipStream_t s, bool *direct_written) {
-    std::vector<char> host(f->ks.xy_bytes);
-    HIP_TRY(hipMemcpyAsync(host.data(), inv->launch.xy.get(), host.size(), hipMemcpyDeviceToHost, s));
+static int run_natives(mmhip_invocation *inv, mmhip_filter *f, HArgs &a, hipStream_t s, bool *direct_written) {
+    const std::vector<char> &host = inv->pro_records;
+    if ((int)host.size() != f->ks.xy_bytes) return fail("internal: no prologue records for this launch");
     NativeDirectOut direct;
-    if (direct_output(f, a, s, &direct) != 0) return -1;
+    if (inv->pro_own_pixels == 1 && direct_output_wanted(f, a)) {
+        direct.out = a.out;
+        direct.row_stride = a.row_stride;
+        direct.first_row = a.first_row;
+        direct.num_rows = a.num_rows;
+        direct.region_x = a.region_x;
+        direct.region_w = a.region_width;
+    }
     inv->ws.env.supersampling = f->kopt.supersampling;
     inv->ws.env.edge_x = f->kopt.edge_x;
     inv->ws.env.edge_y = f->kopt.edge_y;
@@ -1046,6 +1100,7 @@
         NativeEntry &e = inv->natives[k];
         HNativeRec rec = call.rec;
         if (e.map && (e.w != a.render_width || e.h != a.render_height)) {
+            ++inv->host_waits;
             HIP_TRY(hipDeviceSynchronize());
             drop_native_map(inv, k, &table_changed);
         }
@@ -1097,11 +1152,13 @@
         for (const RecordedCall &call : calls) used[call.k] = 1;
         for (size_t k = (size_t)f->ks.native_sites; k < f->ks.natives.size(); ++k) {
             if (used[k] || !inv->natives[k].map) continue;
+            ++inv->host_waits;
             HIP_TRY(hipStreamSynchronize(s));
             drop_native_map(inv, k, &table_changed);
         }
     }
-    if (table_changed && upload_image_table(inv, s) != 0) return -1;
+    if (table_changed && upload_table_slot(inv, s) != 0) return -1;
+    point_at_tables(inv, a);
     return 0;
 }
 
@@ -1222,11 +1279,8 @@
     a.floatmap = floatmap;
     a.edge_color_x = inv->edge_color_x;
     a.edge_color_y = inv->edge_color_y;
-    a.uservals = inv->d_uv.get<HUserval>();
-    a.images = inv->d_images.get<HImageDesc>();
+    point_at_tables(inv, a);
     a.num_images = (uint32_t)inv->images.size();
-    a.curves = inv->d_curves.get();
-    a.gradients = inv->d_gradients.get();
     a.out = out_device;
     a.native_slot_base = inv->native_slot_base;
     return a;
@@ -1245,7 +1299,7 @@
 
     HArgs a = render_args(inv, frame, t, region_x, region_y, region_w, region_h, first_row, last_row, out_device, row_stride, bpp, floatmap);
     const size_t rowtab_bytes = inv->launch.rowtab.bytes;
-    if (grow_launch_buffers(inv->launch, f->ks, region_w, a.num_rows, f->ks.row_values > 0, s) != 0) return -1;
+    if (grow_launch_buffers(inv, inv->launch, f->ks, region_w, a.num_rows, f->ks.row_values > 0, s) != 0) return -1;
     if (inv->launch.rowtab.bytes != rowtab_bytes) inv->pro_filter = nullptr;
     a.xtab = inv->launch.xtab.get<float>();
     a.ytab = inv->launch.ytab.get<float>();
@@ -1258,21 +1312,34 @@
         key.out = nullptr;
         key.row_stride = key.output_bpp = key.floatmap = key.ppt = 0;
         key.tiles_magic = 0;
-        if (!f->ks.prologue_uses_time) { key.t = 0.0f; key.frame = 0; }
-        const bool fresh = f->ks.natives.empty() && inv->pro_filter == f && inv->pro_stream == (void *)s &&
-                           inv->pro_generation == inv->table_generation &&
-                           memcmp(&key, &inv->pro_args, sizeof key) == 0;
+        const float time_t = f->ks.prologue_uses_time ? a.t : 0.0f;
+        const int time_frame = f->ks.prologue_uses_time ? a.frame : 0;
+        if (!f->ks.prologue_computes_with_time) { key.t = 0.0f; key.frame = 0; }
+        key.uservals = nullptr;
+        key.images = nullptr;
+        key.curves = key.gradients = nullptr;
+        const bool records_fresh = inv->pro_filter == f && inv->pro_stream == (void *)s &&
+                                   inv->pro_generation == inv->table_generation &&
+                                   (!f->ks.prologue_reads_images || inv->pro_input_generation == inv->input_generation) &&
+                                   memcmp(&key, &inv->pro_args, sizeof key) == 0;
+        const bool fresh = records_fresh && memcmp(&time_t, &inv->pro_t, sizeof time_t) == 0 && time_frame == inv->pro_frame;
         if (!fresh) {
+            inv->pro_filter = nullptr;
             int n = std::max(region_w, a.num_rows);
             HIP_TRY(hipModuleLaunchKernel(f->f_pro, (unsigned)((n + 255) / 256), 1, 1, 256, 1, 1, 0, s, params, nullptr));
+            ++inv->prologue_launches;
             if (f->ks.row_values > 0)
                 HIP_TRY(hipModuleLaunchKernel(f->f_rows, (unsigned)((a.num_rows + 255) / 256), 1, 1, 256, 1, 1, 0, s, params, nullptr));
-            if (!f->ks.natives.empty() && run_natives(inv, f, a, s, &direct_written) != 0) return -1;
+            if (!f->ks.natives.empty() && !records_fresh && read_back_prologue(inv, f, a, s) != 0) return -1;
+            inv->pro_t = time_t;
+            inv->pro_frame = time_frame;
             inv->pro_args = key;
             inv->pro_filter = f;
             inv->pro_stream = (void *)s;
             inv->pro_generation = inv->table_generation;
-        }
+            inv->pro_input_generation = inv->input_generation;
+        }
+        if (!f->ks.natives.empty() && run_natives(inv, f, a, s, &direct_written) != 0) return -1;
     }
     const LaunchGeometry geo = launch_geometry(f->ks, region_w, a.num_rows);
     const long nwg = geo.nwg;
@@ -1388,6 +1455,7 @@
         HIP_TRY(hipMemcpyAsync(xt.data(), a.xtab, xt.size() * sizeof(float), hipMemcpyDeviceToHost, s));
         HIP_TRY(hipMemcpyAsync(yt.data(), a.ytab, yt.size() * sizeof(float), hipMemcpyDeviceToHost, s));
     }
+    ++inv->host_waits;
     HIP_TRY(hipStreamSynchronize(s));
     if (cc.direct_ok < 0) cc.direct_ok = ask_direct && samples_own_pixels(a, xt, yt) ? 1 : 0;
     auto frame_by_frame = [&]() -> int {
@@ -1461,7 +1529,10 @@
     HIP_TRY(nb.work.grow(jobs_max * (ck_bytes + map_bytes), idle));
     HIP_TRY(nb.maps.grow(kept * map_bytes, idle));
     HIP_TRY(nb.tables.grow(tables_bytes, idle));
-    if (nb.uploaded_pending) HIP_TRY(hipEventSynchronize(nb.uploaded));
+    if (nb.uploaded_pending) {
+        ++inv->host_waits;
+        HIP_TRY(hipEventSynchronize(nb.uploaded));
+    }
     nb.uploaded_pending = false;
     HIP_TRY(nb.host.grow(tables_bytes));
     {
@@ -1591,13 +1662,16 @@
     const int slots = per_frame ? per_batch : 1;
     if (rowtab_stride * slots > (size_t)INT32_MAX || xy_stride * slots > (size_t)INT32_MAX)
         return fail("render_clip: the batch's row tables are too large; lower MMHIP_CLIP_MAX_FRAMES");
-    if (grow_launch_buffers(inv->launch, f->ks, region_w, num_rows, false, s) != 0) return -1;
+    if (grow_launch_buffers(inv, inv->launch, f->ks, region_w, num_rows, false, s) != 0) return -1;
     inv->pro_filter = nullptr;
-    auto wait = [s] { return hipStreamSynchronize(s); };
+    auto wait = [inv, s] { ++inv->host_waits; return hipStreamSynchronize(s); };
     HIP_TRY(inv->clip.xy.grow(xy_stride * slots, wait, true));
     if (rows) HIP_TRY(inv->clip.rowtab.grow(rowtab_stride * slots * sizeof(float), wait));
     ClipBuffers::Table &tab = inv->clip.table[inv->clip.next_table++ & 1];
-    if (tab.pending) HIP_TRY(hipEventSynchronize(tab.uploaded));
+    if (tab.pending) {
+        ++inv->host_waits;
+        HIP_TRY(hipEventSynchronize(tab.uploaded));
+    }
     tab.pending = false;
     const size_t tab_bytes = (size_t)num_frames * sizeof(HClipFrame);
     HIP_TRY(tab.host.grow(tab_bytes));
@@ -1781,6 +1855,7 @@
     int rc = mmhip_render(inv, frame, t, 0, 0, inv->render_w, inv->render_h, 0, inv->render_h, d, inv->render_w * 4, 4, 0,
                           nullptr);
     if (rc == 0) {
+        inv->host_waits += 2;
         hipError_t e = hipStreamSynchronize(inv->stream);
         if (e == hipSuccess) e = hipMemcpy(out_rgba, d, bytes, hipMemcpyDeviceToHost);
         if (e != hipSuccess) rc = fail(std::string("render: ") + hipGetErrorString(e));
diff --git a/mathmap_amd/csrc/runtime_internal.h b/mathmap_amd/csrc/runtime_internal.h
--- a/mathmap_amd/csrc/runtime_internal.h
+++ b/mathmap_amd/csrc/runtime_internal.h
@@ -101,6 +101,19 @@
     }
 };
 
+struct TableRing {
+    enum { SLOTS = 4 };
+    struct Slot {
+        DeviceBuffer dev;
+        PinnedBuffer host;
+        hipEvent_t done = nullptr;
+        bool pending = false;
+        ~Slot() { if (done) (void)hipEventDestroy(done); }
+    } slot[SLOTS];
+    int cur = -1;
+    size_t off_uv = 0, off_curves = 0, off_gradients = 0, bytes = 0;
+};
+
 struct ClipBuffers {
     DeviceBuffer xy, rowtab;
     struct Table {
@@ -152,7 +165,7 @@
     std::vector<int> image_slot_of_uv;
     std::vector<float> curves;
     std::vector<uint32_t> gradients;
-    DeviceBuffer d_uv, d_images, d_curves, d_gradients;
+    TableRing tables;
     int native_slot_base = 0;
     bool tables_dirty = true;
     std::vector<DeviceBuffer> owned;
@@ -172,10 +185,17 @@
     long direct_native_launches = 0;
     long tolerance_blur_launches = 0;
     mm::HArgs pro_args{};
+    float pro_t = 0.0f;
+    int pro_frame = 0;
     const mmhip_filter *pro_filter = nullptr;
     void *pro_stream = nullptr;
     unsigned long long pro_generation = 0, table_generation = 1;
     unsigned long long input_generation = 1;
+    std::vector<char> pro_records;
+    int pro_own_pixels = -1;
+    unsigned long long pro_input_generation = 0;
+    long host_waits = 0;
+    long prologue_launches = 0;
     LaunchBuffers launch;
     ClipBuffers clip;
     long clip_batched_launches = 0;
```

After: 425,300. About the same (-0.3%).
